# grayhong/self-diagnosing-gan

Measured on AMD Instinct MI355X. Metric: images/sec (G+D step), higher is better.
Workload: dtype f32

## Files before the change

### include/diagan_hip.h

```cpp
#ifndef DIAGAN_HIP_H
#define DIAGAN_HIP_H
#include <stddef.h>
#include <stdint.h>
#ifdef __cplusplus
extern "C" {
#endif

#define DIAGAN_OK 0
#define DIAGAN_EINVAL (-1)
#define DIAGAN_EHIP (-2)
#define DIAGAN_EUNSUP (-3)

const char* diagan_last_error(void);
int diagan_abi_version(void);
const char* diagan_target_arch(void);


int diagan_ldr_scores_f64(const double* rec, int T, int64_t N, int64_t row_stride, double* ldr,
                          double* ldrd, double* ldrv, double* ldrm, const double* t_vals, int n_t,
                          double* conf, double floor_val, double ratio, void* workspace,
                          void* stream);

int diagan_ldr_scores_f32(const float* rec, int T, int64_t N, int64_t row_stride, float* ldr,
                          float* ldrd, float* ldrv, float* ldrm, const float* t_vals, int n_t,
                          float* conf, float floor_val, float ratio, void* workspace, void* stream);

int diagan_logit_scatter(const float* logit, const int64_t* idx, int64_t n, void* rec_row,
                         int64_t N, int out_is_f64, int* oob_counter, void* stream);



int diagan_conv_gemm(const float* x, const float* w, float* y, const float* bias,
                     const float* residual, int res_relu, const float* mask_src, float mask_slope,
                     const float* pro_scale, const float* pro_shift, int pro_mode, float out_scale,
                     const float* scale0, const float* scale1, int scale_split,
                     int B, int Hi, int Wi, int Ci, int Ho, int Wo, int Co, int R, int S, int sy,
                     int dr, int off, int up, int Kp, int tile_cfg, float* splitk_ws, int64_t splitk_ws_floats,
                     float* stat_partials, int pro_group_rows, void* stream);
int diagan_conv_gemm_pick_ksplit(int M, int Co, int Kp, int cfg);

int diagan_conv3x3_co4_supported(int Ci, int Co, int R, int S, int sy, int dr, int off, int up);
int diagan_conv3x3_co4(const float* x, const float* w, float* y, const float* bias, const float* residual,
                       const float* pro_scale, const float* pro_shift, int pro_mode, int B, int H, int W, int Ci,
                       int dr, int off, int Kp, int group_imgs, void* stream);

int diagan_conv3x3_ci4_supported(int Ci, int Co, int R, int S, int sy, int dr, int off, int up);
int diagan_conv3x3_ci4(const float* x, const float* w, float* y, const float* bias, float out_scale, const float* scale0,
                       const float* scale1, int scale_split, int B, int H, int W, int Co, int Kp, void* stream);

int diagan_conv3x3_co4_wgrad_supported(int Ci, int Co, int R, int S, int sy, int dr, int off, int up);
int diagan_conv3x3_co4_wgrad_splits(int B, int H);
int diagan_conv3x3_co4_wgrad(const float* dy, const float* x, float* slab, int64_t slab_stride, int64_t bias_off,
                             const float* pro_scale, const float* pro_shift, int pro_mode, int B, int H, int W,
                             int Ci, int Kp, void* stream);

int diagan_conv_gemm_pick_cfg(int M, int Co, int Kp, int allow_split);
int diagan_conv_gemm_tile_rows(int cfg);
int diagan_conv_gemm_tile_cols(int cfg);
int diagan_conv_wino_supported(int Hi, int Wi, int Ci, int Ho, int Wo, int Co, int R, int S, int sy, int dr, int off,
                               int up);
int diagan_conv_wino_pool_supported(int B, int Hi, int Wi, int Ci, int Ho, int Wo, int Co, int R, int S, int sy, int dr,
                                    int off, int up, int pro_mode, int64_t ws_floats);
int diagan_conv_wino_unpool_supported(int B, int Hi, int Wi, int Ci, int Ho, int Wo, int Co, int R, int S, int sy, int dr,
                                      int off, int up, int64_t ws_floats);
int diagan_conv_gemm_set_wino(int mode);
int diagan_conv_gemm_get_wino(void);
int diagan_conv_gemm_set_wino4(int mode);
int diagan_conv_gemm_set_wino4x(int mode);
int diagan_conv_gemm_get_wino4x(void);
int diagan_conv_gemm_set_splitk_fused(int mode);
int diagan_conv_gemm_set_splitk_tickets(int* buf, int64_t slots);
typedef struct diagan_conv_opts {
  int32_t wino, wino4, wino4x, gemm_x3, gemm_x3b, splitk_fused, force_ksplit, tune;
  int32_t* tickets;
  int64_t ticket_slots;
} diagan_conv_opts;
int diagan_conv_gemm_next_opts(const diagan_conv_opts* opts);
int diagan_conv_gemm_pending_opts(diagan_conv_opts* opts);
int diagan_conv_gemm_last_cfg(void);
int diagan_conv_gemm_set_x3(int mode);
int diagan_conv_gemm_get_x3(void);
int diagan_conv_gemm_set_x3b(int mode);
int diagan_conv_gemm_get_x3b(void);
int diagan_conv_gemm_set_x3_pieces(int n);
int diagan_conv_gemm_get_x3_pieces(void);
int diagan_conv_gemm_x3b_force_form(int form);
int diagan_conv_gemm_out_map(int mul, int offy, int offx, int y0, int y1, int x0, int x1, int OH, int OW);
int diagan_conv_gemm_final_cfg(int B, int Hi, int Wi, int Ci, int Ho, int Wo, int Co, int R, int S, int sy, int dr, int off, int up,
                               int Kp, int allow_split, int64_t ws_floats, int pro_group_rows, int pro_mode, int plain_epilogue,
                               int want_stats);
int diagan_conv_wino4_pool_used(int B, int Ho, int Wo, int Ci, int Co, int64_t ws_floats);
int diagan_conv_wino4_upin_supported(int B, int Hi, int Wi, int Ci, int Ho, int Wo, int Co, int R, int S, int sy, int dr,
                                     int off, int up, int64_t ws_floats, int pro_group_rows);
int diagan_conv_gemm_weights_hint(const float* u, int kind, int flip, float scale);
int diagan_conv_gemm_last_weight_format(int* kind, int* flip, float* scale, int64_t* floats, int64_t* launches);
int64_t diagan_wino_weight_blocks(int Co, int Ci);
int diagan_wino_weights_batched(const void* jobs, int n, int blocks, void* stream);
int diagan_conv_gemm_pick_cfg_geom(int B, int Hi, int Wi, int Ci, int Ho, int Wo, int Co, int R, int S, int sy, int dr,
                                   int off, int up, int Kp, int allow_split, int64_t ws_floats);
int diagan_conv_gemm_pick_cfg_grouped(int B, int Hi, int Wi, int Ci, int Ho, int Wo, int Co, int R, int S, int sy, int dr,
                                      int off, int up, int Kp, int allow_split, int64_t ws_floats, int pro_group_rows);
int diagan_conv_gemm_set_stamp_buffer(unsigned long long* buf, int64_t slots);
int diagan_conv_gemm_tune(int force_ksplit, int flags, int lds_delta_bytes);

int diagan_conv_wgrad(const float* dy, const float* x, float* slab, int splits, int segments, int64_t slab_stride,
                      int64_t bias_off, const float* pro_scale, const float* pro_shift, int pro_mode, int B, int Hi, int Wi, int Ci, int Ho,
                      int Wo, int Co, int R, int S, int sy, int dr, int off, int up, int Kp,
                      void* stream);
int diagan_conv_wgrad_splits(int M, int Co, int Kp);
typedef struct {
  const float* dy;
  const float* x;
  float* slab;
  const float* pro_scale;
  const float* pro_shift;
  int64_t slab_stride, bias_off;
  int32_t splits, segments, pro_mode, B, Hi, Wi, Ci, Ho, Wo, Co, R, S, sy, dr, off, up, Kp, pad_;
} diagan_wgrad_job;
int diagan_conv_wgrad_batched(const diagan_wgrad_job* jobs, int n, void* stream);
int diagan_conv_wgrad_batch_max(void);
int diagan_conv_wgrad_batch_class(int Hi, int Wi, int Ci, int Ho, int Wo, int Co, int R, int S, int sy, int dr, int off, int up,
                                  int Kp, int pro_mode);
int diagan_conv_wgrad_uses_wino(int Hi, int Wi, int Ci, int Ho, int Wo, int Co, int R, int S, int sy, int dr, int off,
                                int up, int Kp);
int diagan_conv_wgrad_splits_geom(int B, int Hi, int Wi, int Ci, int Ho, int Wo, int Co, int R, int S, int sy, int dr,
                                  int off, int up, int Kp);
int diagan_conv_wgrad_uses_x3(int B, int Hi, int Wi, int Ci, int Ho, int Wo, int Co, int R, int S, int sy, int dr, int off,
                              int up, int Kp, int pro_mode, int64_t bias_off);
int diagan_conv_wgrad_set_x3(int on);

typedef struct {
  float* slab[2];
  const float* u[2];
  const float* v[2];
  const float* state[2];
  double* partials[2];
  float* grad;
  const float* W;
  int64_t stride;
  int splits, n_elem, n_w, Kp;
  int nctx, first_block;
} diagan_wgrad_layer;
int diagan_wgrad_finish_batched(const void* table_dev, int n_layers, int64_t total_blocks, int any_sn, void* stream);
int diagan_wgrad_finish_block_elems(int splits);

int diagan_wgrad_reduce(const float* slab, int splits, int64_t n_elem, float* out, int accumulate,
                        const float* w, double* dot_partials, void* stream);


int diagan_sn_power_iter(const float* W, float* u_buffer, float* sigma_buffer, float* u_out,
                         float* v_out, float* state, float* work, int Co, int Kp, float eps,
                         int update_buffers, void* stream);

typedef struct {
  const float* W;
  float* u_buf;
  float* sigma_buf;
  float* u_out;
  float* v_out;
  float* state;
  float* work;
  float* Wf;
  float* Wd;
  int Co, Ci, RS, Kp, Kd, pad;
} diagan_sn_layer;
int diagan_sn_prepare_batched(const void* table_dev, int n_layers, int max_Co, int max_Ci, int max_RS,
                              int max_Kp, float eps, int update_buffers, int write_wd, void* stream);
int diagan_pack_batched(const void* table_dev, int n_layers, int max_Co, int max_Ci, int max_RS, int write_wd,
                        void* stream);

int diagan_pack_weights(const float* W, const float* inv_sigma, float* Wf, float* Wd, int Co, int Ci,
                        int RS, int Kp, int Kd, void* stream);
int diagan_pack_oihw(const float* w, float scale, float* Wf, float* Wd, int Co_src, int Ci_src, int R, int S, int Co, int Ci, int Kp,
                     int Kd, void* stream);
int diagan_unpack_oihw(const float* gWp, float scale, float* gw, int Co_src, int Ci_src, int R, int S, int Ci, int Kp, void* stream);
int diagan_parity_weights(const float* w, float* buf, float* gw, int n, int R, int S, int C, int Kp, const int* kp, const int* off,
                          int adjoint, void* stream);


int diagan_sn_grad_fix(const float* G, const double* dot_partials, int nparts, const float* u,
                       const float* v, const float* state, float* grad, int Co, int Kp,
                       int accumulate, void* stream);


int diagan_nchw_to_nhwc(const float* src, float* dst, int B, int C, int H, int W, int Cp, void* stream);
int diagan_nhwc_to_nchw(const float* src, float* dst, int B, int C, int H, int W, int Cp, void* stream);

int diagan_tanh_fwd(const float* x, float* y, int64_t n, void* stream);
int diagan_tanh_bwd(const float* y, const float* g, float* gx, int64_t n, void* stream);

int64_t diagan_colred_workspace(int64_t M, int C);

int diagan_bn_stats(const float* x, int64_t M, int C, const float* gamma, const float* beta, float eps,
                    float momentum, float* running_mean, float* running_var, int training,
                    float* mean_out, float* invstd_out, float* scale_out, float* shift_out,
                    void* workspace, void* stream);
int diagan_bn_stats_grouped(const float* x, int64_t M, int C, int groups, const float* gamma, const float* beta, float eps,
                            float momentum, float* running_mean, float* running_var, float* mean_out, float* invstd_out,
                            float* scale_out, float* shift_out, void* workspace, void* stream);

int diagan_bn_stats_fused(const float* partials, int tiles, int64_t M, int C, const float* gamma, const float* beta,
                          float eps, float momentum, float* running_mean, float* running_var, float* mean_out,
                          float* invstd_out, float* scale_out, float* shift_out, int groups, double* workspace,
                          int64_t workspace_doubles, void* stream);
int diagan_bn_stats_fused_splits(int tiles, int C, int groups);

int diagan_bn_bwd(const float* g, const float* x, int64_t M, int C, const float* scale, const float* shift,
                  const float* mean, const float* invstd, int batch_stats, int relu, float slope,
                  const float* drop, float drop_scale, float* dgamma, float* dbeta,
                  int accumulate_param_grads, const float* residual, float* dx, float* coef,
                  void* workspace, void* stream);

int diagan_colsum(const float* x, int64_t M, int C, float* out, int accumulate, void* workspace, void* stream);

int diagan_upsample2x(const float* x, float* out, int B, int H, int W, int C, int pro_mode,
                      const float* scale, const float* shift, int group_imgs, void* stream);
int diagan_upsample2x_bwd(const float* g, float* out, int B, int H, int W, int C, const float* residual,
                          void* stream);

int diagan_avgpool2(const float* x, float* out, int B, int H, int W, int C, const float* residual, int relu_in,
                    void* stream);
int diagan_boxsum2(const float* x, float* out, int B, int H, int W, int C, int relu_in, void* stream);
int diagan_avgpool2_bwd(const float* g, float* out, int B, int H, int W, int C, const float* residual,
                        void* stream);

int diagan_head_fwd(const float* x, const float* w, const float* inv_sigma, const float* inv_sigma1, int split_b,
                    const float* bias, float* pooled, float* logit, int B, int HW, int C, void* stream);
int diagan_head_bwd(const float* dlogit, const float* w, const float* inv_sigma, const float* inv_sigma1, int split_b,
                    const float* x, const float* pooled, float* gx, float* G, double* dot, float* dbias,
                    int accumulate_bias, int B, int HW, int C, void* stream);

int diagan_act_fwd(const float* x, const float* scale, const float* shift, float slope, const float* drop, float drop_scale,
                   float* out, int64_t M, int C, void* stream);
int diagan_act_bwd(const float* g, const float* x, float slope, const float* drop, float drop_scale, float* out, int64_t n,
                   void* stream);
int diagan_linear1_fwd(const float* x, const float* w, const float* bias, float* logit, int B, int C, void* stream);
int diagan_linear1_wgrad(const float* dlogit, const float* x, float* dw, float* dbias, int B, int C, void* stream);
int diagan_linear1_bwd_input(const float* dlogit, const float* w, float* gx, int B, int C, void* stream);

int diagan_add(const float* a, const float* b, float* out, int64_t n, void* stream);


int diagan_loss_dis(const float* out_real, int n_real, const float* out_fake, int n_fake, int loss_type,
                    int gold, float* d_real, float* d_fake, float* out3, void* stream);
int diagan_loss_gen(const float* out_fake, int n, int k, int loss_type, float* d_fake, float* out1, void* stream);

int diagan_adam_step(float* p, const float* g, float* m, float* v, int64_t n, float lr, float beta1,
                     float beta2, float eps, float bias_correction1, float bias_correction2_sqrt, float grad_scale,
                     void* stream);
int diagan_adam_step_dev(float* p, const float* g, float* m, float* v, int64_t n, const float* hyper8, void* stream);

typedef struct diagan_ctx diagan_ctx;
int diagan_comm_unique_id(void* id128);
int diagan_ctx_create(diagan_ctx** out, const void* id128, int rank, int world, int device);
int diagan_ctx_destroy(diagan_ctx* ctx);
int diagan_ctx_rank(const diagan_ctx* ctx);
int diagan_ctx_world(const diagan_ctx* ctx);
int diagan_allreduce_grads(diagan_ctx* ctx, float* slab, int64_t n, void* stream);
int diagan_allgather_logits(diagan_ctx* ctx, const void* send, void* recv, int64_t n_per_rank, int elem_bytes,
                            void* stream);


int diagan_fused_bias_act(const float* x, const float* bias, const float* refer, float* out, int64_t n,
                          int64_t step_b, int size_b, int act, int grad, float alpha, float scale, void* stream);

int diagan_styled_bias_act(const float* x, const float* demod, const float* noise, const float* strength,
                           const float* bias, float* out, int B, int P, int C, int noise_per_image, float alpha,
                           float scale, void* stream);

int diagan_rowdot_chunks(int B, int P);
int diagan_rowdot(const float* a, const float* b, float* out, float* workspace, int B, int P, int C, void* stream);
int diagan_styled_bias_act_bwd(const float* gy, const float* y, const float* x, const float* demod, const float* noise,
                               float* gx, float* work_d, float* work_b, float* work_s, int B, int P, int C,
                               int noise_per_image, float alpha, float scale, void* stream);
int diagan_styled_bias_act_bwd_finish(const float* work_d, const float* work_b, const float* work_s, float* gd, float* gb, float* gs, int B,
                                      int P, int C, void* stream);

int diagan_small_linear_fwd(const float* x, const float* W, const float* bias, float* out, int B, int K, int C, float scale, float bias_mul,
                            void* stream);
int diagan_small_linear_bwd(const float* g, const float* x, const float* W, float* gW, float* gbias, float* gx, int B, int K, int C,
                            float scale, float bias_mul, void* stream);
int diagan_demod_fwd(const float* s, const float* w, float* d, float* wsq, int B, int Ci, int Co, int taps, float scale2, float eps,
                     void* stream);
int diagan_demod_bwd(const float* gd, const float* d, const float* s, const float* w, const float* wsq, float* gw, float* gs, int B, int Ci,
                     int Co, int taps, float scale2, void* stream);

int diagan_styled_bias_act_mod(const float* x, const float* demod, const float* noise, const float* strength, const float* bias,
                               const float* post, float* out, float* out_mod, int B, int P, int C, int noise_per_image, float alpha,
                               float scale, void* stream);
int diagan_styled_bias_act_mod_bwd(const float* gy, const float* gmod, const float* post, const float* y, const float* x,
                                   const float* demod, const float* noise, float* gx, float* work_d, float* work_b, float* work_s,
                                   float* work_p, int B, int P, int C, int noise_per_image, float alpha, float scale, void* stream);

int diagan_torgb_fwd(const float* x, const float* s, const float* w, const float* bias, float* out, int B, int P, int C, void* stream);
int diagan_torgb_bwd(const float* gy, const float* x, const float* s, const float* w, float* gx, float* work, float* gs, float* gw, int B,
                     int P, int C, void* stream);
int diagan_fromrgb_fwd(const float* x, const float* w, const float* bias, float* y, int B, int P, int C, float wscale, float alpha,
                       float scale, void* stream);
int diagan_fromrgb_bwd(const float* gy, const float* y, const float* x, const float* w, float* gx, float* work, int B, int P, int C,
                       float wscale, float alpha, float scale, void* stream);
int diagan_bias_act_fir(const float* input, const float* bias, const float* kernel, float* out, int major, int in_h, int in_w, int minor,
                        int kernel_h, int kernel_w, int pad_x0, int pad_x1, int pad_y0, int pad_y1, float alpha, float scale,
                        void* stream);
int diagan_bias_act_gate_bwd(const float* gy, const float* z, const float* bias, float* gx, float* work_b, int B, int P, int C,
                             float alpha, float scale, void* stream);
int diagan_fir_gate_bwd(const float* g, const float* kernel, const float* ref, const float* bias, float* gz, float* work_b, int major,
                        int in_h, int in_w, int minor, int kernel_h, int kernel_w, int pad_x0, int pad_x1, int pad_y0, int pad_y1,
                        float alpha, float scale, void* stream);
int diagan_upfirdn2d_add(const float* input, const float* kernel, const float* addend, float* out, int major, int in_h, int in_w, int minor,
                         int kernel_h, int kernel_w, int up_x, int up_y, int down_x, int down_y, int pad_x0, int pad_x1, int pad_y0,
                         int pad_y1, void* stream);
int diagan_bias_act_add(const float* x, const float* bias, const float* addend, float* out, int64_t n, int C, float alpha, float scale,
                        void* stream);
int diagan_fir_styled_act(const float* input, const float* kernel, float* out, int major, int in_h, int in_w, int minor, int kernel_h,
                          int kernel_w, int pad_x0, int pad_x1, int pad_y0, int pad_y1, const float* demod, const float* noise,
                          const float* strength, const float* bias, const float* post, int noise_per_image, float alpha, float scale,
                          void* stream);


int diagan_upfirdn2d(const float* input, const float* kernel, float* out, int major, int in_h, int in_w, int minor,
                     int kernel_h, int kernel_w, int up_x, int up_y, int down_x, int down_y, int pad_x0, int pad_x1,
                     int pad_y0, int pad_y1, int* out_h, int* out_w, void* stream);

int diagan_row_sqnorm(const float* x, float* out, int N, int D, int ld, void* stream);
int diagan_kth_smallest_rows(const float* T, const float* row_add, int rows, int cols, int ld, int k, float* out,
                             void* stream);
int diagan_any_lt_rows(const float* T, const float* row_add, const float* thr_col, const float* thr_row, int rows,
                       int cols, int ld, float* out, void* stream);
int diagan_any_lt_cols(const float* T, const float* row_add, const float* thr_col, const float* thr_row, int rows,
                       int cols, int ld, float* out, void* stream);

int diagan_gemm_f64(const double* A, const double* B, double* C, int M, int N, int K, int lda, int ldb, int ldc, int trans_a,
                    double alpha, double beta, double diag, double* trace_part, void* stream);
int diagan_gemm_f64_tile(void);
int diagan_sum_f64(const double* x, int64_t n, int square, double* out, void* stream);
int diagan_trace_f64(const double* S, int D, int ld, double* out, void* stream);
int diagan_sym_f64(double* S, int D, int ld, double scale, void* stream);
int diagan_scale_diag_f64(const double* src, double* dst, int D, int ld, double alpha, double d, void* stream);
int diagan_fid_term(const double* mu1, const double* mu2, const double* S1, const double* S2, int D, int ld, double* out,
                    void* stream);
int diagan_feat_colsum_chunks(int N);
int diagan_feat_moments(const void* x, int x_f64, int N, int D, int ld, double* mask, double* part, double* count, double* mean,
                        void* stream);
int diagan_feat_center(const void* x, int x_f64, const double* mask, const double* mean, int N, int D, int ld, double* xc, int ldc,
                       void* stream);
int diagan_moments_merge(double* n_run, double* mean_run, double* m2_run, int ld, const double* n_b, const double* mean_b,
                         const double* m2_b, int ldb, int D, void* stream);


int diagan_augment_params(void);
int diagan_augment_workspace(int B, int H, int W, int pad_x1, int pad_x2, int pad_y1, int pad_y2, int backward, int64_t* bytes);
int diagan_augment_forward(const float* img, const double* params, int B, int H, int W, int pad_x1, int pad_x2, int pad_y1,
                           int pad_y2, float* out, void* workspace, void* stream);
int diagan_augment_backward(const float* gout, const double* params, int B, int H, int W, int pad_x1, int pad_x2, int pad_y1,
                            int pad_y2, float* gimg, void* workspace, void* stream);

int diagan_incep_conv_kp(int R, int S, int Ci);
int diagan_incep_conv(const float* x, int B, int H, int W, int ctot_in, int c0_in, int Ci, const float* w, const float* bias, int Co,
                      int R, int S, int Kp, int stride_h, int stride_w, int pad_h, int pad_w, float* y, int Ho, int Wo, int ctot_out,
                      int c0_out, int relu, void* stream);
int diagan_incep_pool3(const float* x, int B, int H, int W, int ctot_in, int c0_in, int C, float* y, int Ho, int Wo, int ctot_out,
                       int c0_out, int mode, void* stream);
int diagan_incep_gap(const float* x, int B, int HW, int C, float* y, void* stream);
int diagan_incep_prep(const float* x, int nhwc, int B, int H, int W, float* y, int Ho, int Wo, int resize, float a, float b,
                      void* stream);

int diagan_poly_mmd_ws(int m);
int diagan_poly_mmd_sums(const void* X, int x_f64, int Nx, int ldx, const void* Y, int y_f64, int Ny, int ldy, const int* idx_x,
                         const int* idx_y, int S, int m, int D, int degree, double gamma, double coef0, double* ws, double* out,
                         void* stream);
int diagan_is_ws(int N, int C, int splits);
int diagan_is_scores(const float* logits, int N, int C, int ld, int splits, double* ws, double* out, void* stream);

int diagan_nn_argmin(const float* q, int Nq, int ldq, const float* c, int Nc, int ldc, const float* c_sqnorm, int D, long idx_offset,
                     int accumulate, float* best_t, long* best_idx, void* ws, void* stream);
size_t diagan_nn_argmin_ws(int Nq, int Nc);

#ifdef __cplusplus
}
#endif
#endif
```

### self-diagnosing-gan_amd/csrc/conv_gemm.hip

```cpp
#include "conv_common.h"
#include "switches.h"
#include <type_traits>
#include <stdlib.h>
#include <string.h>

extern "C" int diagan_conv_gemm_tile_rows(int cfg);
extern "C" int diagan_conv_gemm_tile_cols(int cfg);
extern "C" int diagan_conv_gemm_pick_ksplit(int M, int Co, int Kp, int cfg);
extern "C" int diagan_conv_gemm_pick_cfg_geom(int B, int Hi, int Wi, int Ci, int Ho, int Wo, int Co, int R, int S, int sy,
                                              int dr, int off, int up, int Kp, int allow_split, int64_t ws_floats);
extern "C" int diagan_conv_gemm_pick_cfg_grouped(int B, int Hi, int Wi, int Ci, int Ho, int Wo, int Co, int R, int S, int sy,
                                                 int dr, int off, int up, int Kp, int allow_split, int64_t ws_floats,
                                                 int pro_group_rows);
extern "C" int diagan_conv_wino_supported(int Hi, int Wi, int Ci, int Ho, int Wo, int Co, int R, int S, int sy, int dr,
                                          int off, int up);

namespace diagan {
int launch_gemm_x3(const ConvGemmArgs& a, float* ws, hipStream_t st);
bool gemm_x3_geom_ok(const ConvGemmArgs& a);
long gemm_x3_ws_floats(int Co, int Kp);
int launch_gemm_x3b(const ConvGemmArgs& a, const OutMap& map, float* ws, hipStream_t st);
bool gemm_x3b_geom_ok(const ConvGemmArgs& a);
long gemm_x3b_ws_floats(int Co, int Kp);
void gemm_x3b_force_form(int form);
int launch_wino(ConvGemmArgs a, float* ws, hipStream_t st);
long wino_ws_floats(int Co, int Ci);
int wino_ksplit(int B, int Ho, int Wo, int Ci, int Co, int allow_split, long ws_floats, int min_wgs);
int launch_wino4(ConvGemmArgs a, float* ws, hipStream_t st);
long wino4_ws_floats(int Co, int Ci);
bool wino4_geom_ok(int Ho, int Wo, int Ci);
int wino4_ksplit(int B, int Ho, int Wo, int Ci, int Co, int allow_split, long ws_floats);
bool wino4_pool_ok(int B, int Ho, int Wo, int Ci, int Co, long ws_floats, bool force);
int launch_wino4_pool(ConvGemmArgs a, float* ws, hipStream_t st);
int launch_wino4_unpool(ConvGemmArgs a, float* ws, hipStream_t st);
bool wino4_upin_ok(int B, int Ho, int Wo, int Ci, int Co, long ws_floats, bool force);
int launch_wino_weights_batched(const WinoJob* jobs, int n, int blocks, hipStream_t st);
int launch_wino4_upin(ConvGemmArgs a, float* ws, hipStream_t st);
void wino4_set_x3(int mode);
int wino4_get_x3();
int launch_wino_pool(ConvGemmArgs a, float* ws, hipStream_t st);
int launch_wino_unpool(ConvGemmArgs a, float* ws, hipStream_t st);
int wino_pool_ksplit(int B, int Ho, int Wo, int Ci, int Co, long slab_floats, int min_wgs);


template <int BM, int BN, int WM, int WN, int BK = 32, int PRO = -1, bool STAMP = false, bool FP = false, int KG = 1>
__global__ __launch_bounds__(256 * KG) void conv_gemm_kernel(const ConvGemmArgs a) {
  constexpr int CH = BK / 4;
  constexpr int RP = 256 / CH;
  constexpr int TM = BM / WM / 32, TN = BN / WN / 32;
  constexpr int AJ = BM / RP, BJ = BN / RP;
  auto swz = [](int row, int q) {
    return BK == 64 ? (q ^ (row & 15)) : BK == 32 ? (q ^ ((row >> 1) & 7)) : (q ^ ((row >> 2) & 3));
  };
  static_assert(WM * WN == 4, "4 waves");
  extern __shared__ __attribute__((aligned(16))) float smem_all[];
  constexpr int STAGE_FLOATS = 2 * (BM + BN) * BK;
  const int kg = KG > 1 ? __builtin_amdgcn_readfirstlane((int)threadIdx.x >> 8) : 0;
  float* const smem = smem_all + kg * STAGE_FLOATS;
  float* As = smem;
  float* Bs = smem + 2 * BM * BK;

  unsigned long long st_t[6] = {0, 0, 0, 0, 0, 0}, st_r0 = 0;
  auto stamp = [&](int i) {
    if constexpr (STAMP) {
      __builtin_amdgcn_sched_barrier(0);
      st_t[i] = __builtin_amdgcn_s_memtime();
      __builtin_amdgcn_sched_barrier(0);
    }
  };
  if constexpr (STAMP) st_r0 = __builtin_amdgcn_s_memrealtime();
  if (a.tune & 1) __builtin_amdgcn_s_setprio(3);
  stamp(0);
  const ConvGeom& g = a.g;
  const int pro_mode = PRO >= 0 ? PRO : a.pro_mode;
  const int tid = KG > 1 ? (threadIdx.x & 255) : threadIdx.x, lane = tid & 63, wave = tid >> 6;
  const int wm = wave / WN, wn = wave % WN;
  const int tiles_n = (g.Co + BN - 1) / BN;
  const int nwg = gridDim.x;
  const int tile = xcd_remap(blockIdx.x, nwg);
  const int m0 = (tile / tiles_n) * BM, n0 = (tile % tiles_n) * BN;

  const int lrow = tid / CH, lq = tid % CH;
  const int ush = g.up >> 1, upm = g.up - 1;
  const int pstep = (g.Ci * 4) >> ush;
  int base[AJ];
  unsigned vmask[AJ];
#pragma unroll
  for (int j = 0; j < AJ; ++j) {
    const int m = m0 + lrow + RP * j;
    base[j] = 0;
    vmask[j] = 0;
    if (m < a.M) {
      const unsigned t = fdiv((unsigned)m, a.dWo);
      const int ox = m - (int)t * g.Wo;
      const unsigned b = fdiv(t, a.dHo);
      const int oy = (int)t - (int)b * g.Ho;
      const int iy0 = oy * g.sy + g.off, ix0 = ox * g.sy + g.off;
      base[j] = (int)b * g.Hi * g.Wi * g.Ci * 4 + (iy0 * g.Wi + ix0) * pstep;
      unsigned mk = 0;
      if (g.up == 1) {
        const int ylo = g.dr > 0 ? max(0, -iy0) : max(0, iy0 - g.Hi + 1);
        const int yhi = g.dr > 0 ? min(g.R - 1, g.Hi - 1 - iy0) : min(g.R - 1, iy0);
        const int xlo = g.dr > 0 ? max(0, -ix0) : max(0, ix0 - g.Wi + 1);
        const int xhi = g.dr > 0 ? min(g.S - 1, g.Wi - 1 - ix0) : min(g.S - 1, ix0);
        if (yhi >= ylo) mk |= (2u << yhi) - (1u << ylo);
        if (xhi >= xlo) mk |= ((2u << xhi) - (1u << xlo)) << 16;
      } else {
        for (int r = 0; r < g.R; ++r) {
          const int yn = iy0 + r * g.dr;
          if (yn >= 0 && (yn & upm) == 0 && (yn >> ush) < g.Hi) mk |= 1u << r;
        }
        for (int q = 0; q < g.S; ++q) {
          const int xn = ix0 + q * g.dr;
          if (xn >= 0 && (xn & upm) == 0 && (xn >> ush) < g.Wi) mk |= 0x10000u << q;
        }
      }
      vmask[j] = mk;
    }
  }
  const int nk_all = g.Kp / BK;
  const int k_per = (nk_all + a.ksplit * KG - 1) / (a.ksplit * KG);
  const int k_begin = min((int)(blockIdx.y * KG + kg) * k_per, nk_all), k_end = min(k_begin + k_per, nk_all);
  int kc, kr, ks;
  {
    const int kflat = k_begin * BK + lq * 4, tap = kflat / g.Ci;
    kc = kflat - tap * g.Ci;
    kr = tap / g.S;
    ks = tap - kr * g.S;
  }
  const int rowstep = g.dr * g.Wi * pstep, colstep = g.dr * pstep;

  const __amdgpu_buffer_rsrc_t xsrc = __builtin_amdgcn_make_buffer_rsrc(
      const_cast<float*>(a.x), 0, (int)((unsigned)g.B * g.Hi * g.Wi * g.Ci * 4u), 0x00020000);
  const __amdgpu_buffer_rsrc_t wsrc = __builtin_amdgcn_make_buffer_rsrc(
      const_cast<float*>(a.w), 0, (int)((unsigned)g.Co * g.Kp * 4u), 0x00020000);
  const bool affine = pro_mode == PRO_AFFINE_RELU || pro_mode == PRO_AFFINE;
  const int pro_group_off = a.pro_group_rows > 0 ? (m0 / a.pro_group_rows) * g.Ci : 0;
  unsigned wbase[BJ];
#pragma unroll
  for (int j = 0; j < BJ; ++j) wbase[j] = ((unsigned)(n0 + lrow + RP * j) * g.Kp + lq * 4) * 4u;

  f32x4 ra[AJ], rb[BJ], psc = {1.f, 1.f, 1.f, 1.f}, psh = {0.f, 0.f, 0.f, 0.f};
  unsigned a_ok = 0;

  const bool ut = (g.Ci % BK) == 0;
  int ukr = 0, uks = 0, ukc = 0;
  unsigned avo[AJ], tap_ok = 0;
  auto tap_setup = [&]() {
    const int toff = ukr * rowstep + uks * colstep + lq * 16;
    const int r_ = min(ukr, 15), s_ = 16 + uks;
    tap_ok = 0;
#pragma unroll
    for (int j = 0; j < AJ; ++j) {
      const unsigned okb = (vmask[j] >> r_) & (vmask[j] >> s_) & 1u;
      avo[j] = (unsigned)(base[j] + toff) | ((okb ^ 1u) << 31);
      tap_ok |= okb << j;
    }
  };
  if (ut) {
    const int kflat0 = k_begin * BK, tap0 = kflat0 / g.Ci;
    ukc = kflat0 - tap0 * g.Ci;
    ukr = tap0 / g.S;
    uks = tap0 - ukr * g.S;
    tap_setup();
  }
  const float* const pro_sc_lane = a.pro_scale ? a.pro_scale + pro_group_off + lq * 4 : nullptr;
  const float* const pro_sh_lane = a.pro_shift ? a.pro_shift + pro_group_off + lq * 4 : nullptr;

  int tapoff = 0, krs = 0, kss = 0;
  auto load_piece = [&](int kk, int p, auto utc) {
    if constexpr (decltype(utc)::value) {
      if (p == 0) {
        a_ok = tap_ok;
        if (affine) {
          psc = *reinterpret_cast<const f32x4*>(pro_sc_lane + ukc);
          psh = *reinterpret_cast<const f32x4*>(pro_sh_lane + ukc);
        }
      }
      if (p < AJ) {
        ra[p] = __builtin_bit_cast(f32x4, __builtin_amdgcn_raw_buffer_load_b128(xsrc, avo[p], ukc * 4, 0));
      } else {
        rb[p - AJ] = __builtin_bit_cast(f32x4, __builtin_amdgcn_raw_buffer_load_b128(wsrc, wbase[p - AJ], kk * (BK * 4), 0));
      }
      if (p == AJ + BJ - 1) {
        ukc += BK;
        if (ukc >= g.Ci) {
          ukc = 0;
          if (++uks == g.S) {
            uks = 0;
            ++ukr;
          }
          tap_setup();
        }
      }
      return;
    }
    if (p == 0) {
      tapoff = kr * rowstep + ks * colstep + kc * 4;
      krs = min(kr, 15);
      kss = 16 + ks;
      a_ok = 0;
      if (affine) {
        const int kcs = min(kc, g.Ci - 4);
        psc = *reinterpret_cast<const f32x4*>(a.pro_scale + pro_group_off + kcs);
        psh = *reinterpret_cast<const f32x4*>(a.pro_shift + pro_group_off + kcs);
      }
    }
    if (p < AJ) {
      const int j = p;
      const unsigned okb = (vmask[j] >> krs) & (vmask[j] >> kss) & 1u;
      const unsigned off = (unsigned)(base[j] + tapoff) | ((okb ^ 1u) << 31);
      ra[j] = __builtin_bit_cast(f32x4, __builtin_amdgcn_raw_buffer_load_b128(xsrc, off, 0, 0));
      a_ok |= okb << j;
    } else {
      const int j = p - AJ;
      rb[j] = __builtin_bit_cast(f32x4, __builtin_amdgcn_raw_buffer_load_b128(wsrc, wbase[j] + (unsigned)kk * (BK * 4u), 0, 0));
    }
    if (p == AJ + BJ - 1) {
      kc += BK;
      if (g.Ci >= BK) {
        const bool w = kc >= g.Ci;
        kc -= w ? g.Ci : 0;
        ks += w ? 1 : 0;
        const bool r = ks == g.S;
        ks = r ? 0 : ks;
        kr += r ? 1 : 0;
      } else {
        const int kflat = (kk + 1) * BK + lq * 4, tap = kflat / g.Ci;
        kc = kflat - tap * g.Ci;
        kr = tap / g.S;
        ks = tap - kr * g.S;
      }
    }
  };
  auto load_tiles = [&](int kk) {
    if (ut) {
#pragma unroll
      for (int p = 0; p < AJ + BJ; ++p) load_piece(kk, p, std::true_type{});
    } else {
#pragma unroll
      for (int p = 0; p < AJ + BJ; ++p) load_piece(kk, p, std::false_type{});
    }
  };
  auto store_piece = [&](int buf, int p) {
    if (p < AJ) {
      const int j = p;
      const int row = lrow + RP * j;
      f32x4 v = ra[j];
      if (pro_mode != PRO_NONE) {
        if (affine) v = v * psc + psh;
        if (pro_mode == PRO_LRELU) {
#pragma unroll
          for (int e = 0; e < 4; ++e) v[e] = v[e] > 0.f ? v[e] : 0.2f * v[e];
        } else if (pro_mode != PRO_AFFINE) {
#pragma unroll
          for (int e = 0; e < 4; ++e) v[e] = fmaxf(v[e], 0.f);
        }
        if (affine) {
          const float keep = (float)((a_ok >> j) & 1u);
          v *= keep;
        }
      }
      *reinterpret_cast<f32x4*>(As + buf * BM * BK + row * BK + (swz(row, lq) << 2)) = v;
    } else {
      const int j = p - AJ;
      const int row = lrow + RP * j;
      *reinterpret_cast<f32x4*>(Bs + buf * BN * BK + row * BK + (swz(row, lq) << 2)) = rb[j];
    }
  };
  auto store_tiles = [&](int buf) {
#pragma unroll
    for (int p = 0; p < AJ + BJ; ++p) store_piece(buf, p);
  };

  f32x16 acc[TM][TN];
#pragma unroll
  for (int i = 0; i < TM; ++i)
#pragma unroll
    for (int j = 0; j < TN; ++j)
#pragma unroll
      for (int e = 0; e < 16; ++e) acc[i][j][e] = 0.f;

  const int fi = lane & 31, fh = lane >> 5;
  int fao[BK / 8], fbo[BK / 8];
#pragma unroll
  for (int u = 0; u < BK / 8; ++u) {
    const int ra_ = wm * (TM * 32) + fi, rb_ = wn * (TN * 32) + fi;
    fao[u] = ra_ * BK + (swz(ra_, 2 * u + fh) << 2);
    fbo[u] = 2 * BM * BK + rb_ * BK + (swz(rb_, 2 * u + fh) << 2);
  }
  const int sto = lrow * BK + (swz(lrow, lq) << 2);

  stamp(1);
  if (k_begin < k_end) {
    load_tiles(k_begin);
    store_tiles(0);
  }
  __syncthreads();

  constexpr int NE = (BK / 8) * 4, NP = AJ + BJ;
  constexpr int PPE = (2 * NP + NE - 1) / NE;
  constexpr int LE = (NP + PPE - 1) / PPE;
  static_assert(2 * LE <= NE, "load and store pieces of a tile must not share an e-step");
  auto kstep = [&](int kk, auto has_next) {
    const int cur = (kk - k_begin) & 1;
    const float* Ac = As + cur * BM * BK;
    const float* Bc = Bs + cur * BN * BK;
    f32x4 fa[2][TM], fb[2][TN];
    auto read_frags = [&](int slot, int u) {
      const int q = 2 * u + fh;
#pragma unroll
      for (int i = 0; i < TM; ++i) {
        const int row = wm * (TM * 32) + i * 32 + fi;
        fa[slot][i] = *reinterpret_cast<const f32x4*>(Ac + row * BK + (swz(row, q) << 2));
      }
#pragma unroll
      for (int j = 0; j < TN; ++j) {
        const int row = wn * (TN * 32) + j * 32 + fi;
        fb[slot][j] = *reinterpret_cast<const f32x4*>(Bc + row * BK + (swz(row, q) << 2));
      }
    };
    if constexpr (FP) read_frags(0, 0);
#pragma unroll
    for (int u = 0; u < BK / 8; ++u) {
      const int fs = FP ? (u & 1) : 0;
      if constexpr (FP) {
        if (u + 1 < BK / 8) read_frags((u + 1) & 1, u + 1);
      } else {
        read_frags(0, u);
      }
#pragma unroll
      for (int e = 0; e < 4; ++e) {
        const int es = u * 4 + e;
        if (decltype(has_next)::value && es < LE) {
#pragma unroll
          for (int pp = 0; pp < PPE; ++pp)
            if (es * PPE + pp < NP) load_piece(kk + 1, es * PPE + pp, std::false_type{});
        }
        if (decltype(has_next)::value && es >= NE - LE) {
          __builtin_amdgcn_sched_barrier(0);
#pragma unroll
          for (int pp = 0; pp < PPE; ++pp)
            if ((es - (NE - LE)) * PPE + pp < NP) store_piece(cur ^ 1, (es - (NE - LE)) * PPE + pp);
        }
#pragma unroll
        for (int i = 0; i < TM; ++i)
#pragma unroll
          for (int j = 0; j < TN; ++j)
            acc[i][j] = __builtin_amdgcn_mfma_f32_32x32x2f32(fa[fs][i][e], fb[fs][j][e], acc[i][j], 0, 0, 0);
      }
    }
    __syncthreads();
  };
  auto kstep_u = [&](int kk, auto curc, auto has_next) {
    constexpr int cur = decltype(curc)::value;
    f32x4 fa[2][TM], fb[2][TN];
    auto read_frags = [&](int slot, int u) {
#pragma unroll
      for (int i = 0; i < TM; ++i) fa[slot][i] = *reinterpret_cast<const f32x4*>(smem + fao[u] + cur * BM * BK + i * 32 * BK);
#pragma unroll
      for (int j = 0; j < TN; ++j) fb[slot][j] = *reinterpret_cast<const f32x4*>(smem + fbo[u] + cur * BN * BK + j * 32 * BK);
    };
    auto store_piece_u = [&](int p) {
      if (p < AJ) {
        f32x4 v = ra[p];
        if (pro_mode != PRO_NONE) {
          if (affine) v = v * psc + psh;
          if (pro_mode == PRO_LRELU) {
#pragma unroll
            for (int e = 0; e < 4; ++e) v[e] = v[e] > 0.f ? v[e] : 0.2f * v[e];
          } else if (pro_mode != PRO_AFFINE) {
#pragma unroll
            for (int e = 0; e < 4; ++e) v[e] = fmaxf(v[e], 0.f);
          }
          if (affine) {
            const float keep = (float)((a_ok >> p) & 1u);
            v *= keep;
          }
        }
        *reinterpret_cast<f32x4*>(smem + sto + (cur ^ 1) * BM * BK + p * RP * BK) = v;
      } else {
        *reinterpret_cast<f32x4*>(smem + sto + 2 * BM * BK + (cur ^ 1) * BN * BK + (p - AJ) * RP * BK) = rb[p - AJ];
      }
    };
    if constexpr (FP) read_frags(0, 0);
#pragma unroll
    for (int u = 0; u < BK / 8; ++u) {
      const int fs = FP ? (u & 1) : 0;
      if constexpr (FP) {
        if (u + 1 < BK / 8) read_frags((u + 1) & 1, u + 1);
      } else {
        read_frags(0, u);
      }
#pragma unroll
      for (int e = 0; e < 4; ++e) {
        const int es = u * 4 + e;
        if (decltype(has_next)::value && es < LE) {
#pragma unroll
          for (int pp = 0; pp < PPE; ++pp)
            if (es * PPE + pp < NP) load_piece(kk + 1, es * PPE + pp, std::true_type{});
        }
        if (decltype(has_next)::value && es >= NE - LE) {
          __builtin_amdgcn_sched_barrier(0);
#pragma unroll
          for (int pp = 0; pp < PPE; ++pp)
            if ((es - (NE - LE)) * PPE + pp < NP) store_piece_u((es - (NE - LE)) * PPE + pp);
        }
#pragma unroll
        for (int i = 0; i < TM; ++i)
#pragma unroll
          for (int j = 0; j < TN; ++j)
            acc[i][j] = __builtin_amdgcn_mfma_f32_32x32x2f32(fa[fs][i][e], fb[fs][j][e], acc[i][j], 0, 0, 0);
      }
    }
    __syncthreads();
  };
  if (a.tune & 1) __builtin_amdgcn_s_setprio(0);
  stamp(2);
  if (ut) {
    const std::integral_constant<int, 0> b0;
    const std::integral_constant<int, 1> b1;
    int kk = k_begin;
    for (; kk + 2 < k_end; kk += 2) {
      kstep_u(kk, b0, std::true_type{});
      kstep_u(kk + 1, b1, std::true_type{});
    }
    if (kk + 1 < k_end) {
      kstep_u(kk, b0, std::true_type{});
      kstep_u(kk + 1, b1, std::false_type{});
    } else if (kk < k_end) {
      kstep_u(kk, b0, std::false_type{});
    }
  } else {
    for (int kk = k_begin; kk + 1 < k_end; ++kk) kstep(kk, std::true_type{});
    if (k_begin < k_end) kstep(k_end - 1, std::false_type{});
  }
  stamp(3);
  if (a.tune & 2) __builtin_amdgcn_s_setprio(3);
  if constexpr (KG > 1) {
    if (kg > 0) {
#pragma unroll
      for (int i = 0; i < TM; ++i)
#pragma unroll
        for (int j = 0; j < TN; ++j)
#pragma unroll
          for (int e = 0; e < 16; ++e) smem[((i * TN + j) * 16 + e) * 256 + tid] = acc[i][j][e];
    }
    __syncthreads();
    if (kg > 0) return;
#pragma unroll
    for (int q = 1; q < KG; ++q)
#pragma unroll
      for (int i = 0; i < TM; ++i)
#pragma unroll
        for (int j = 0; j < TN; ++j)
#pragma unroll
          for (int e = 0; e < 16; ++e) acc[i][j][e] += smem_all[q * STAGE_FLOATS + ((i * TN + j) * 16 + e) * 256 + tid];
    static_assert(TM * TN * 16 * 256 <= STAGE_FLOATS, "the accumulators of a K-group fit its stage region");
  }

  const float sc0 = a.scale0 ? a.scale0[0] : a.out_scale, sc1 = a.scale1 ? a.scale1[0] : a.out_scale;
  const int split = a.scale0 ? a.scale_split : 0x7fffffff;
  const unsigned rowbytes = (unsigned)g.Co * 4u;
  const unsigned ybytes = (unsigned)a.M * rowbytes;
  float* ydst = a.ksplit > 1 ? a.slab + (long)blockIdx.y * a.M * g.Co : a.y;
  const __amdgpu_buffer_rsrc_t ysrc = __builtin_amdgcn_make_buffer_rsrc(ydst, 0, (int)ybytes, 0x00020000);
  const __amdgpu_buffer_rsrc_t rsrc = __builtin_amdgcn_make_buffer_rsrc(
      const_cast<float*>(a.residual ? a.residual : a.y), 0, a.residual ? (int)ybytes : 0, 0x00020000);
  const __amdgpu_buffer_rsrc_t msrc = __builtin_amdgcn_make_buffer_rsrc(
      const_cast<float*>(a.mask_src ? a.mask_src : a.y), 0, a.mask_src ? (int)ybytes : 0, 0x00020000);
  const float rfloor = a.res_relu ? 0.f : -__builtin_huge_valf();
  float cs1[TN], cs2[TN];
#pragma unroll
  for (int j = 0; j < TN; ++j) cs1[j] = cs2[j] = 0.f;
  auto epilogue = [&](auto has_res, auto has_mask, auto has_stats, auto raw) {
#pragma unroll
    for (int i = 0; i < TM; ++i) {
#pragma unroll
      for (int j = 0; j < TN; ++j) {
        const int n = n0 + wn * (TN * 32) + j * 32 + fi;
        const bool col_ok = n < g.Co;
        const float bv = (!decltype(raw)::value && a.bias && col_ok) ? a.bias[n] : 0.f;
        const int mrow = m0 + wm * (TM * 32) + i * 32 + 4 * fh;
        const unsigned vbase = col_ok ? ((unsigned)mrow * g.Co + n) * 4u : 0x80000000u;
        float rres[16], rmsk[16];
        if (decltype(has_res)::value) {
#pragma unroll
          for (int e = 0; e < 16; ++e)
            rres[e] = __builtin_bit_cast(float, __builtin_amdgcn_raw_buffer_load_b32(
                                                    rsrc, vbase, (int)(((e & 3) + 8 * (e >> 2)) * rowbytes), 0));
        }
        if (decltype(has_mask)::value) {
#pragma unroll
          for (int e = 0; e < 16; ++e)
            rmsk[e] = __builtin_bit_cast(float, __builtin_amdgcn_raw_buffer_load_b32(
                                                    msrc, vbase, (int)(((e & 3) + 8 * (e >> 2)) * rowbytes), 0));
        }
#pragma unroll
        for (int e = 0; e < 16; ++e) {
          const int k = (e & 3) + 8 * (e >> 2);
          const int soff = (int)(k * rowbytes);
          const float av = acc[i][j][e];
          if (decltype(raw)::value) {
            __builtin_amdgcn_raw_buffer_store_b32(__float_as_uint(av), ysrc, vbase, soff, 0);
            continue;
          }
          const int m = mrow + k;
          float v = fmaf(av, m < split ? sc0 : sc1, bv);
          if (decltype(has_res)::value) v += fmaxf(rres[e], rfloor);
          if (decltype(has_mask)::value) v = rmsk[e] > 0.f ? v : v * a.mask_slope;
          __builtin_amdgcn_raw_buffer_store_b32(__float_as_uint(v), ysrc, vbase, soff, 0);
          if (decltype(has_stats)::value) {
            const float vm = (m < a.M && col_ok) ? v : 0.f;
            cs1[j] += vm;
            cs2[j] = fmaf(vm, vm, cs2[j]);
          }
        }
      }
    }
  };
  {
    using T = std::true_type;
    using F = std::false_type;
    const bool hr = a.residual != nullptr, hm = a.mask_src != nullptr, hs = a.stat_partials != nullptr;
    if (a.ksplit > 1) epilogue(F{}, F{}, F{}, T{});
    else if (hs) { if (hr) epilogue(T{}, F{}, T{}, F{}); else epilogue(F{}, F{}, T{}, F{}); }
    else if (hr && hm) epilogue(T{}, T{}, F{}, F{});
    else if (hr) epilogue(T{}, F{}, F{}, F{});
    else if (hm) epilogue(F{}, T{}, F{}, F{});
    else epilogue(F{}, F{}, F{}, F{});
  }
  if (a.stat_partials) {
    float* red = smem;
#pragma unroll
    for (int j = 0; j < TN; ++j) {
      cs1[j] += __shfl_xor(cs1[j], 32, 64);
      cs2[j] += __shfl_xor(cs2[j], 32, 64);
      if (fh == 0) {
        const int col = wn * (TN * 32) + j * 32 + fi;
        red[(wm * BN + col) * 2 + 0] = cs1[j];
        red[(wm * BN + col) * 2 + 1] = cs2[j];
      }
    }
    __syncthreads();
    if (tid < BN && n0 + tid < g.Co) {
      float t1 = 0.f, t2 = 0.f;
#pragma unroll
      for (int w = 0; w < WM; ++w) { t1 += red[(w * BN + tid) * 2]; t2 += red[(w * BN + tid) * 2 + 1]; }
      float* p = a.stat_partials + (long)(tile / tiles_n) * 2 * g.Co;
      p[n0 + tid] = t1;
      p[g.Co + n0 + tid] = t2;
    }
  }
  if constexpr (STAMP) {
    stamp(4);
    asm volatile("s_waitcnt vmcnt(0)" ::: "memory");
    stamp(5);
    if (tid == 0 && a.stamps) {
      unsigned long long* o = a.stamps + ((size_t)blockIdx.y * gridDim.x + blockIdx.x) * 8;
      o[0] = st_r0;
      o[1] = __builtin_amdgcn_s_memrealtime();
      for (int i = 0; i < 5; ++i) o[2 + i] = st_t[i + 1] - st_t[i];
      o[7] = (unsigned long long)__builtin_amdgcn_s_getreg((31 << 11) | 4) |
             ((unsigned long long)__builtin_amdgcn_s_getreg((31 << 11) | 20) << 32);
    }
  }
}

__global__ __launch_bounds__(256) void splitk_epilogue_kernel(const ConvGemmArgs a) {
  const int C4 = a.g.Co >> 2;
  const long n4 = (long)a.M * C4;
  const float sc0 = a.scale0 ? a.scale0[0] : 1.f, sc1 = a.scale1 ? a.scale1[0] : 1.f;
  for (long i = (long)blockIdx.x * 256 + threadIdx.x; i < n4; i += (long)gridDim.x * 256) {
    const int c4 = (int)(i % C4);
    const int m = (int)(i / C4);
    f32x4 s = reinterpret_cast<const f32x4*>(a.slab)[i];
    for (int k = 1; k < a.ksplit; ++k) s += reinterpret_cast<const f32x4*>(a.slab)[(long)k * n4 + i];
    const float sc = a.scale0 ? (m < a.scale_split ? sc0 : sc1) : a.out_scale;
    s *= sc;
    if (a.bias) s += reinterpret_cast<const f32x4*>(a.bias)[c4];
    if (a.residual) {
      f32x4 r;
      if (a.res_up == 1) {
        const int ox = m % a.g.Wo, q = m / a.g.Wo, oy = q % a.g.Ho, b = q / a.g.Ho;
        r = residual_up2(a.residual, b, oy, ox, a.g.Ho >> 1, a.g.Wo >> 1, a.g.Co, c4 * 4);
      } else if (a.res_up == 2) {
        const int ox = m % a.g.Wo, q = m / a.g.Wo, oy = q % a.g.Ho, b = q / a.g.Ho;
        r = 0.25f * *reinterpret_cast<const f32x4*>(a.residual + (((long)b * (a.g.Ho >> 1) + (oy >> 1)) * (a.g.Wo >> 1) + (ox >> 1)) * a.g.Co + c4 * 4);
      } else {
        r = reinterpret_cast<const f32x4*>(a.residual)[i];
      }
      if (a.res_relu) {
#pragma unroll
        for (int e = 0; e < 4; ++e) r[e] = fmaxf(r[e], 0.f);
      }
      s += r;
    }
    if (a.mask_src) {
      const f32x4 ms = reinterpret_cast<const f32x4*>(a.mask_src)[i];
#pragma unroll
      for (int e = 0; e < 4; ++e) s[e] = ms[e] > 0.f ? s[e] : s[e] * a.mask_slope;
    }
    reinterpret_cast<f32x4*>(a.y)[i] = s;
  }
}

static unsigned long long* g_stamps = nullptr;
static long g_stamp_slots = 0;
static int g_force_ksplit = 0;
static int g_tune_flags = -1;
static long g_lds_delta = 0;
static int g_wino = -1;
static int g_wino4 = -1;
struct WinoFormat { const float* u; int kind, flip; float scale; long floats; };
static thread_local WinoFormat g_hint_next = {nullptr, 0, 0, 0.f, 0}, g_hint_now = {nullptr, 0, 0, 0.f, 0}, g_fmt_last = {nullptr, 0, 0, 0.f, 0};
static thread_local long g_weight_launches = 0;
constexpr int kDefaultTune = 0;

static int g_gemm_x3 = -1;
static int g_gemm_x3b = -1;
static int x3b_min_tiles() { return kGemmX3bMinTiles.env(); }
static thread_local OutMap g_map_next = {0, 0, 0, 0, 0, 0, 0, 0, 0};
struct CallOpts {
  int wino, wino4, wino4x, gemm_x3, gemm_x3b, splitk_fused, force_ksplit, tune;
  int* tickets;
  long ticket_slots;
};
static const CallOpts kNoOpts = {-1, -1, -1, -1, -1, -1, 0, -1, nullptr, 0};
static thread_local CallOpts g_opts_next = kNoOpts, g_opts_now = kNoOpts;
static thread_local int g_last_cfg = 0;
int call_opt_wino4x() { return g_opts_now.wino4x; }
static int sel_wino() { return kWino.get(g_opts_now.wino, g_wino); }
static int sel_wino4() { return g_opts_now.wino4 >= 0 ? g_opts_now.wino4 : g_wino4; }
static int sel_force_ksplit() { return g_opts_now.force_ksplit > 0 ? g_opts_now.force_ksplit : g_force_ksplit; }
static bool gemm_x3_on() { return kGemmX3.get(g_opts_now.gemm_x3, g_gemm_x3) != 0; }
static bool gemm_x3b_on() { return kGemmX3b.get(g_opts_now.gemm_x3b, g_gemm_x3b) != 0; }
static bool x3b_takes(const ConvGemmArgs& a, int cfg, int64_t ws_floats) {
  if (!gemm_x3b_on() || !(cfg == 1 || cfg == 3 || cfg == 5 || cfg == 7 || cfg == 8)) return false;
  const ConvGeom& g = a.g;
  return gemm_x3b_geom_ok(a) && g.Kp >= 128 && g.Co >= 64 && (long)cdiv(a.M, 128) * cdiv(g.Co, 128) >= x3b_min_tiles() &&
         (double)a.M * g.Co * g.Kp >= 4e9 && gemm_x3b_ws_floats(g.Co, g.Kp) <= ws_floats;
}
static int g_splitk_fused = -1;
static int* g_tickets = nullptr;
static long g_ticket_slots = 0;
static int* splitk_tickets(long tiles) {
  if (!kSplitkFused.get(g_opts_now.splitk_fused, g_splitk_fused)) return nullptr;
  if (g_opts_now.tickets) return tiles <= g_opts_now.ticket_slots ? g_opts_now.tickets : nullptr;
  return (g_tickets && tiles <= g_ticket_slots) ? g_tickets : nullptr;
}

static int splitk_second_stage(const ConvGemmArgs& a, hipStream_t st, const char* what) {
  long blocks = ((long)a.M * (a.g.Co / 4) + 255) / 256;
  if (blocks > 4096) blocks = 4096;
  hipLaunchKernelGGL(splitk_epilogue_kernel, dim3((int)blocks), dim3(256), 0, st, a);
  return check_launch(what);
}

template <int BM, int BN, int WM, int WN, int BK, int PRO, bool STAMP = false, bool FP = false, int KG = 1>
static int launch_one(const ConvGemmArgs& a, hipStream_t st) {
  const int tiles = cdiv(a.M, BM) * cdiv(a.g.Co, BN);
  const size_t lds = (size_t)((long)((size_t)2 * KG * (BM + BN) * BK * sizeof(float)) + g_lds_delta);
  auto kern = conv_gemm_kernel<BM, BN, WM, WN, BK, PRO, STAMP, FP, KG>;
  static FuncAttrLatch latch;
  DG_LDS(latch, kern, lds);
  hipLaunchKernelGGL(kern, dim3(tiles, a.ksplit), dim3(256 * KG), lds, st, a);
  return a.ksplit > 1 ? splitk_second_stage(a, st, "conv_gemm") : check_launch("conv_gemm");
}

template <int BM, int BN, int WM, int WN, int BK = 32, bool SPEC = false, bool FP = false, int KG = 1>
static int launch_cfg(const ConvGemmArgs& a, hipStream_t st) {
  if (a.stamps && KG > 1) return set_err(DIAGAN_EUNSUP, "conv_gemm: no stamped build of the two-group kernel");
  if (a.stamps) {
    if (a.pro_mode == PRO_NONE) return launch_one<BM, BN, WM, WN, BK, PRO_NONE, true, FP>(a, st);
    if (a.pro_mode == PRO_RELU) return launch_one<BM, BN, WM, WN, BK, PRO_RELU, true, FP>(a, st);
    return set_err(DIAGAN_EUNSUP, "conv_gemm: the stamped diagnostic kernels exist for prologue modes 0 and 1");
  }
  if (SPEC)
    return with_pro(a.pro_mode, [&](auto pro) { return launch_one<BM, BN, WM, WN, BK, SPEC ? decltype(pro)::value : -1, false, FP, KG>(a, st); });
  return launch_one<BM, BN, WM, WN, BK, -1, false, FP, KG>(a, st);
}

}

using namespace diagan;

static bool split128_enabled() { return kSplit128.env() > 0; }

DIAGAN_API int diagan_conv_gemm_pick_cfg(int M, int Co, int Kp, int allow_split) {
  const int small = 7;
  if (Kp <= 256) return small;
  const long t128 = (long)cdiv(M, 128) * cdiv(Co, 128), t64 = (long)cdiv(M, 64) * cdiv(Co, 64);
  if (split128_enabled() && allow_split && (Co & 127) == 0 && t128 <= 256 && diagan_conv_gemm_pick_ksplit(M, Co, Kp, 1) > 1) return 1;
  if (Co <= 64 && Kp >= 256) return M >= 65536 ? 5 : (M >= 32768 ? 8 : 7);
  const long s128 = 256 * 2, s64 = 256 * 4;
  const double q128 = (double)t128 / (double)(cdiv(t128, s128) * s128);
  const double q64 = (double)t64 / (double)(cdiv(t64, s64) * s64);
  const double waste128 = (double)M * Co / ((double)t128 * 128 * 128);
  const double waste64 = (double)M * Co / ((double)t64 * 64 * 64);
  const double bias = 1.08;
  if (bias * q128 * waste128 > q64 * waste64) return 1;
  if (kKg2.env() && t64 <= 256 && Kp >= 16 * 32 && diagan_conv_gemm_pick_ksplit(M, Co, Kp, small) == 1) return 14;
  return small;
}

DIAGAN_API int diagan_conv_gemm_pick_ksplit(int M, int Co, int Kp, int cfg) {
  const int forced = sel_force_ksplit() > 0 ? sel_force_ksplit() : kKsplit.env();
  if (forced > 0 && !(Co & 3)) return forced < Kp / 64 ? forced : (Kp / 64 > 0 ? Kp / 64 : 1);
  if (Co & 3) return 1;
  const int nk = Kp / 32;
  if (cfg == 1) {
    if (!split128_enabled()) return 1;
    const long t128 = (long)cdiv(M, 128) * cdiv(Co, 128);
    if (t128 > 256 || nk < 64) return 1;
    int s = t128 <= 128 ? 4 : 2;
    while (s > 1 && nk / s < 16) --s;
    return s;
  }
  if (cfg != 3 && cfg != 7) return 1;
  const long tiles = (long)cdiv(M, 64) * cdiv(Co, 64);
  if (nk < 16) return 1;
  if (tiles <= 320) {
    if (nk < 64) return 1;
    int s = nk / 24;
    return s > 4 ? 4 : s;
  }
  if (tiles > 512) return 1;
  long sp = 1024 / tiles;
  if (sp > nk / 8) sp = nk / 8;
  return sp < 2 ? 1 : (int)sp;
}

const float* diagan::wino_weights_ready(int kind, int flip, float scale, long floats) {
  g_fmt_last = WinoFormat{nullptr, kind, flip, scale, floats};
  if (g_hint_now.u && g_hint_now.kind == kind && g_hint_now.flip == flip && g_hint_now.scale == scale) return g_hint_now.u;
  ++g_weight_launches;
  return nullptr;
}

DIAGAN_API int diagan_conv_gemm_weights_hint(const float* u, int kind, int flip, float scale) {
  g_hint_next = WinoFormat{u, kind, flip, scale, 0};
  return DIAGAN_OK;
}
DIAGAN_API int diagan_conv_gemm_last_weight_format(int* kind, int* flip, float* scale, int64_t* floats, int64_t* launches) {
  if (kind) *kind = g_fmt_last.kind;
  if (flip) *flip = g_fmt_last.flip;
  if (scale) *scale = g_fmt_last.scale;
  if (floats) *floats = g_fmt_last.floats;
  if (launches) *launches = g_weight_launches;
  return DIAGAN_OK;
}
DIAGAN_API int64_t diagan_wino_weight_blocks(int Co, int Ci) { return (int64_t)cdiv(Ci, 32) * cdiv(Co, 64); }
DIAGAN_API int diagan_wino_weights_batched(const void* jobs, int n, int blocks, void* stream) {
  DG_REQUIRE(jobs && n > 0 && blocks > 0, "wino_weights_batched: bad job table");
  return launch_wino_weights_batched((const WinoJob*)jobs, n, blocks, (hipStream_t)stream);
}

DIAGAN_API int diagan_conv_gemm(const float* x, const float* w, float* y, const float* bias,
                                const float* residual, int res_relu, const float* mask_src, float mask_slope,
                                const float* pro_scale, const float* pro_shift, int pro_mode,
                                float out_scale, const float* scale0, const float* scale1, int scale_split,
                                int B, int Hi, int Wi, int Ci, int Ho, int Wo, int Co,
                                int R, int S, int sy, int dr, int off, int up, int Kp, int tile_cfg,
                                float* splitk_ws, int64_t splitk_ws_floats, float* stat_partials, int pro_group_rows,
                                void* stream) {
  g_hint_now = g_hint_next;
  g_hint_next = WinoFormat{nullptr, 0, 0, 0.f, 0};
  g_fmt_last = WinoFormat{nullptr, 0, 0, 0.f, 0};
  const OutMap map = g_map_next;
  g_map_next = OutMap{0, 0, 0, 0, 0, 0, 0, 0, 0};
  struct OptsScope {
    OptsScope() { g_opts_now = g_opts_next; g_opts_next = kNoOpts; }
    ~OptsScope() { g_opts_now = kNoOpts; }
  } opts_scope;
  g_last_cfg = 0;
  DG_REQUIRE(x && w && y, "conv_gemm: null tensor");
  DG_REQUIRE(B > 0 && Hi > 0 && Wi > 0 && Ho > 0 && Wo > 0 && Co > 0 && R > 0 && S > 0, "conv_gemm: bad dims");
  DG_REQUIRE(Ci > 0 && (Ci & 3) == 0, "conv_gemm: Ci=%d must be a positive multiple of 4 (pad the tensor)", Ci);
  DG_REQUIRE(up == 1 || up == 2, "conv_gemm: up=%d unsupported (1 or 2)", up);
  DG_REQUIRE(dr == 1 || dr == -1, "conv_gemm: dr must be +-1");
  DG_REQUIRE(R <= 15 && S <= 15, "conv_gemm: filter %dx%d larger than 15x15", R, S);
  DG_REQUIRE(Kp % 32 == 0 && Kp >= R * S * Ci, "conv_gemm: Kp=%d must be a multiple of 32 and >= R*S*Ci=%d", Kp, R * S * Ci);
  DG_REQUIRE(pro_mode >= 0 && pro_mode <= 4, "conv_gemm: bad pro_mode %d", pro_mode);
  DG_REQUIRE(!(pro_mode == PRO_AFFINE_RELU || pro_mode == PRO_AFFINE) || (pro_scale && pro_shift),
             "conv_gemm: affine prologue needs scale/shift");
  DG_REQUIRE((long)B * Ho * Wo * Co * 4 < (1L << 31) && (long)B * Hi * Wi * Ci * 4 < (1L << 31) &&
                 (long)Co * Kp * 4 < (1L << 31),
             "conv_gemm: tensors must be smaller than 2 GiB (32-bit buffer offsets)");
  ConvGemmArgs a;
  a.x = x; a.w = w; a.y = y; a.bias = bias; a.residual = residual; a.mask_src = mask_src;
  a.pro_scale = pro_scale; a.pro_shift = pro_shift; a.mask_slope = mask_slope; a.out_scale = out_scale;
  a.scale0 = scale0; a.scale1 = scale1; a.scale_split = scale_split;
  DG_REQUIRE(!scale0 || scale1, "conv_gemm: scale0 and scale1 must be given together");
  DG_REQUIRE(!(stat_partials && mask_src), "conv_gemm: stat_partials (forward statistics) and mask_src (backward mask) are exclusive");
  a.pro_mode = pro_mode; a.M = B * Ho * Wo; a.res_relu = res_relu & 1; a.res_up = (res_relu & 2) ? 1 : (res_relu & 4) ? 2 : 0;
  DG_REQUIRE((res_relu & ~7) == 0 && (res_relu & 6) != 6, "conv_gemm: res_relu=%d (bit 0: relu(residual), bit 1: half-resolution residual, "
             "up-sampled; bit 2: half-resolution residual, un-pooled)", res_relu);
  DG_REQUIRE(a.res_up != 1 || (residual && !(Ho & 1) && !(Wo & 1) && !mask_src && !a.res_relu),
             "conv_gemm: a half-resolution residual needs the tensor, even Ho / Wo, no backward mask and no ReLU on it");
  DG_REQUIRE(a.res_up != 2 || (residual && !(Ho & 1) && !(Wo & 1) && !a.res_relu && !stat_partials),
             "conv_gemm: an un-pooled half-resolution residual needs the tensor, even Ho / Wo, no ReLU on it, no statistics");
  a.g = ConvGeom{B, Hi, Wi, Ci, Ho, Wo, Co, R, S, sy, dr, off, up, R * S * Ci, Kp};
  a.dWo = make_fastdiv((unsigned)Wo);
  a.dHo = make_fastdiv((unsigned)Ho);
  a.stat_partials = stat_partials;
  a.pro_group_rows = pro_group_rows;
  hipStream_t st = (hipStream_t)stream;
  int cfg = tile_cfg != 0 ? tile_cfg
                          : diagan_conv_gemm_pick_cfg_grouped(B, Hi, Wi, Ci, Ho, Wo, Co, R, S, sy, dr, off, up, Kp,
                                                              (splitk_ws && !stat_partials) ? 1 : 0,
                                                              splitk_ws ? splitk_ws_floats : 0, pro_group_rows);
  if (tile_cfg == 0 && splitk_ws && x3b_takes(a, cfg, splitk_ws_floats)) cfg = 17;
  g_last_cfg = cfg;
  if (map.mul != 0) {
    DG_REQUIRE(map.mul > 0 && map.OH > 0 && map.OW > 0 && map.y0 >= 0 && map.x0 >= 0 && map.y1 <= Ho && map.x1 <= Wo &&
                   map.offy >= 0 && map.offx >= 0 && (map.y1 <= map.y0 || map.mul * (map.y1 - 1 - map.y0) + map.offy < map.OH) &&
                   (map.x1 <= map.x0 || map.mul * (map.x1 - 1 - map.x0) + map.offx < map.OW) &&
                   (long)B * map.OH * map.OW * Co * 4 < (1L << 31),
               "conv_gemm: output map (mul %d, off %d/%d, window [%d,%d) x [%d,%d), target %d x %d) does not fit", map.mul, map.offy,
               map.offx, map.y0, map.y1, map.x0, map.x1, map.OH, map.OW);
    DG_REQUIRE(cfg == 17, "conv_gemm: an output map is written by the split-operand kernel only (tile_cfg 17; ask "
               "diagan_conv_gemm_final_cfg first)");
  }
  const int bm = diagan_conv_gemm_tile_rows(cfg);
  DG_REQUIRE(bm > 0, "conv_gemm: unknown tile_cfg %d (0 = auto, 1 = 128x128, 3 = 64x64, 5 = 256x64, 7 = 64x64 with fragment "
             "prefetch, 8 = 128x64 with fragment prefetch, 9 = Winograd F(2x2,3x3), 11 / 12 = Winograd + average pool and its data-gradient, 13 = Winograd F(4x4,3x3), 15 = the same on the bilinear x2 of a half-resolution input; 2, 4, 6, 10 were retired)", tile_cfg);
  DG_REQUIRE(pro_group_rows >= 0 && (pro_group_rows == 0 || (pro_group_rows % bm == 0 && a.M % pro_group_rows == 0)),
             "conv_gemm: pro_group_rows=%d must be a multiple of the %d-row tile and divide M=%d", pro_group_rows, bm, a.M);
  a.slab = splitk_ws;
  a.tickets = nullptr;
  a.ksplit = 1;
  a.tune = first_set(g_opts_now.tune, g_tune_flags, kDefaultTune);
  a.stamps = nullptr;
  if (g_stamps) {
    const long wgs = (long)cdiv(a.M, bm) * cdiv(Co, diagan_conv_gemm_tile_cols(cfg)) * 16;
    DG_REQUIRE(wgs <= g_stamp_slots, "conv_gemm: stamp buffer has %ld slots, this launch may need %ld", g_stamp_slots, wgs);
    a.stamps = g_stamps;
  }
  if (splitk_ws && !stat_partials) {
    const int ks = diagan_conv_gemm_pick_ksplit(a.M, Co, Kp, cfg);
    if (ks > 1 && (int64_t)ks * a.M * Co <= splitk_ws_floats) a.ksplit = ks;
  }
  if (cfg == 11) {
    DG_REQUIRE(diagan_conv_wino_supported(Hi, Wi, Ci, Ho, Wo, Co, R, S, sy, dr, off, up) && dr == 1 && Co % 64 == 0 &&
                   (pro_mode == PRO_NONE || pro_mode == PRO_RELU) && !mask_src && !stat_partials && !a.res_up && pro_group_rows == 0,
               "conv_gemm: tile_cfg 11 (Winograd + average pool) needs a forward 3x3 / stride 1 / pad 1 geometry with even H, W, "
               "Ci %% 8 == 0, Co %% 64 == 0, prologue none / ReLU, no mask, statistics or half-resolution residual");
    if (sel_wino4() != 0 && splitk_ws && wino4_pool_ok(B, Ho, Wo, Ci, Co, (long)splitk_ws_floats, sel_wino4() == 2)) {
      a.ksplit = 1;
      return launch_wino4_pool(a, splitk_ws, st);
    }
    const long wfl = wino_ws_floats(Co, Ci);
    DG_REQUIRE(splitk_ws && splitk_ws_floats >= wfl, "conv_gemm: tile_cfg 11 needs %ld floats of workspace for the transformed weights", wfl);
    int ks = wino_pool_ksplit(B, Ho, Wo, Ci, Co, (long)splitk_ws_floats - wfl, 192);
    if (ks < 1) ks = 1;
    a.ksplit = ks;
    a.slab = splitk_ws + wfl;
    int rc = launch_wino_pool(a, splitk_ws, st);
    if (rc == DIAGAN_OK && ks > 1) {
      ConvGemmArgs e = a;
      e.M = B * (Ho >> 1) * (Wo >> 1);
      e.scale_split = a.scale_split >> 2;
      e.out_scale = a.out_scale;
      rc = splitk_second_stage(e, st, "conv_wino_pool split-K epilogue");
    }
    return rc;
  }
  if (cfg == 12) {
    DG_REQUIRE(diagan_conv_wino_supported(Hi, Wi, Ci, Ho, Wo, Co, R, S, sy, dr, off, up) && dr == -1 && Co % 64 == 0 &&
                   pro_mode == PRO_NONE && !stat_partials && !a.res_up && pro_group_rows == 0,
               "conv_gemm: tile_cfg 12 (data-gradient through an average pool, Winograd) needs the data-gradient geometry of a "
               "3x3 / stride 1 / pad 1 layer with even H, W, Ci %% 8 == 0, Co %% 64 == 0, no prologue, statistics or half-resolution residual");
    if (sel_wino4() != 0 && splitk_ws && wino4_pool_ok(B, Ho, Wo, Ci, Co, (long)splitk_ws_floats, sel_wino4() == 2)) {
      a.ksplit = 1;
      return launch_wino4_unpool(a, splitk_ws, st);
    }
    const long wfl = wino_ws_floats(Co, Ci);
    DG_REQUIRE(splitk_ws && splitk_ws_floats >= wfl, "conv_gemm: tile_cfg 12 needs %ld floats of workspace for the transformed weights", wfl);
    long slab_tiles = ((long)splitk_ws_floats - wfl) / 4;
    int ks = wino_pool_ksplit(B, Ho, Wo, Ci, Co, slab_tiles, 192);
    if (ks < 1) ks = 1;
    a.ksplit = ks;
    a.slab = splitk_ws + wfl;
    int rc = launch_wino_unpool(a, splitk_ws, st);
    if (rc == DIAGAN_OK && ks > 1) rc = splitk_second_stage(a, st, "conv_wino_unpool split-K epilogue");
    return rc;
  }
  if (cfg == 15) {
    DG_REQUIRE(diagan_conv_wino_supported(Hi, Wi, Ci, Ho, Wo, Co, R, S, sy, dr, off, up) && dr == 1 && wino4_geom_ok(Ho, Wo, Ci) &&
                   !mask_src && (pro_group_rows == 0 || pro_group_rows % 512 == 0),
               "conv_gemm: tile_cfg 15 (Winograd F(4x4,3x3) on an up-sampled input) needs a forward 3x3 / stride 1 / pad 1 geometry, "
               "H and W multiples of 4, Ci %% 8 == 0, no backward mask, prologue groups of whole 512-row tiles");
    const long wfl = wino4_ws_floats(Co, Ci);
    DG_REQUIRE(splitk_ws && splitk_ws_floats >= wfl, "conv_gemm: tile_cfg 15 needs %ld floats of workspace for the transformed weights", wfl);
    a.ksplit = 1;
    return launch_wino4_upin(a, splitk_ws, st);
  }
  if (cfg == 13) {
    DG_REQUIRE(diagan_conv_wino_supported(Hi, Wi, Ci, Ho, Wo, Co, R, S, sy, dr, off, up) && wino4_geom_ok(Ho, Wo, Ci),
               "conv_gemm: tile_cfg 13 (Winograd F(4x4,3x3)) needs a 3x3 / stride 1 / pad 1 geometry, H and W multiples of 4, Ci %% 8 == 0");
    const long wfl = wino4_ws_floats(Co, Ci);
    DG_REQUIRE(splitk_ws && splitk_ws_floats >= wfl, "conv_gemm: tile_cfg 13 needs %ld floats of workspace for the transformed weights", wfl);
    int ks = 1;
    if (tile_cfg == 0 && !stat_partials) {
      ks = wino4_ksplit(B, Ho, Wo, Ci, Co, 1, (long)splitk_ws_floats);
      if (ks < 1) ks = 1;
    } else if (sel_force_ksplit() > 1 && !stat_partials && wfl + (long)sel_force_ksplit() * a.M * Co <= splitk_ws_floats && Ci / 8 / sel_force_ksplit() >= 1) {
      ks = sel_force_ksplit();
    }
    a.ksplit = ks;
    a.slab = splitk_ws + wfl;
    int rc = launch_wino4(a, splitk_ws, st);
    if (rc == DIAGAN_OK && ks > 1) rc = splitk_second_stage(a, st, "conv_wino4 split-K epilogue");
    return rc;
  }
  if (cfg == 9) {
    DG_REQUIRE(diagan_conv_wino_supported(Hi, Wi, Ci, Ho, Wo, Co, R, S, sy, dr, off, up),
               "conv_gemm: tile_cfg 9 (Winograd F(2x2,3x3)) needs a 3x3 / stride 1 / pad 1 geometry, even H and W, Ci %% 8 == 0");
    DG_REQUIRE(splitk_ws && splitk_ws_floats >= wino_ws_floats(Co, Ci),
               "conv_gemm: tile_cfg 9 needs %ld floats of workspace for the transformed weights", wino_ws_floats(Co, Ci));
    const long wfl = wino_ws_floats(Co, Ci);
    int ks = 1;
    if (tile_cfg == 0 && !stat_partials) {
      ks = wino_ksplit(B, Ho, Wo, Ci, Co, 1, (long)splitk_ws_floats, 192);
      if (ks < 1) ks = 1;
    } else if (sel_force_ksplit() > 1 && !stat_partials && wfl + (long)sel_force_ksplit() * a.M * Co <= splitk_ws_floats &&
               Ci / 16 / sel_force_ksplit() >= 1) {
      ks = sel_force_ksplit();
    }
    a.ksplit = ks;
    a.slab = splitk_ws + wfl;
    if (ks > 1) a.tickets = splitk_tickets((long)cdiv(a.M / 4, 64) * cdiv(Co, 64));
    int rc = launch_wino(a, splitk_ws, st);
    if (rc == DIAGAN_OK && ks > 1 && !a.tickets) rc = splitk_second_stage(a, st, "conv_wino split-K epilogue");
    return rc;
  }
  DG_REQUIRE(!a.res_up, "conv_gemm: a half-resolution residual is added by the Winograd kernel only (tile_cfg 9; ask "
             "diagan_conv_gemm_pick_cfg_geom first)");
  if (cfg == 16 || (cfg == 14 && tile_cfg == 0 && R == 3 && S == 3 && gemm_x3_on() && gemm_x3_geom_ok(a) && splitk_ws &&
                    gemm_x3_ws_floats(Co, Kp) <= splitk_ws_floats)) {
    DG_REQUIRE(gemm_x3_geom_ok(a) && splitk_ws && gemm_x3_ws_floats(Co, Kp) <= splitk_ws_floats,
               "conv_gemm: tile_cfg 16 (split-operand implicit GEMM) needs stride 1, no up-sampling, Ci %% 32 == 0, an even number of "
               "32-channel K-steps, Kp == R*S*Ci, prologue none / ReLU, no statistics, and %ld floats of workspace", gemm_x3_ws_floats(Co, Kp));
    a.ksplit = 1;
    g_last_cfg = 16;
    return launch_gemm_x3(a, splitk_ws, st);
  }
  if (cfg == 17) {
    DG_REQUIRE(gemm_x3b_geom_ok(a) && splitk_ws && gemm_x3b_ws_floats(Co, Kp) <= splitk_ws_floats,
               "conv_gemm: tile_cfg 17 (split-operand implicit GEMM, 128 x 128 tiles) needs a gather without up-sampling, Ci %% 32 == 0, "
               "Kp == R*S*Ci, prologue none / ReLU / leaky ReLU, a plain epilogue (out_scale, bias, residual) and %ld floats of workspace",
               gemm_x3b_ws_floats(Co, Kp));
    a.ksplit = 1;
    return launch_gemm_x3b(a, map, splitk_ws, st);
  }
  switch (cfg) {
    case 1: return launch_cfg<128, 128, 2, 2, 32, true>(a, st);
    case 3: return launch_cfg<64, 64, 2, 2, 32, true>(a, st);
    case 5: return launch_cfg<256, 64, 4, 1, 32, true>(a, st);
    case 7: return launch_cfg<64, 64, 2, 2, 32, true, true>(a, st);
    case 8: return launch_cfg<128, 64, 2, 2, 32, true, true>(a, st);
    case 14: return launch_cfg<64, 64, 2, 2, 32, true, true, 2>(a, st);
    default: return set_err(DIAGAN_EINVAL, "conv_gemm: unknown tile_cfg %d", tile_cfg);
  }
}

DIAGAN_API int diagan_conv_gemm_tile_rows(int cfg) {
  switch (cfg) { case 1: case 8: case 17: return 128; case 3: case 7: case 14: case 16: return 64; case 5: case 9: case 11: case 12: return 256; case 13: case 15: return 512; default: return 0; }
}
DIAGAN_API int diagan_conv_gemm_tile_cols(int cfg) {
  switch (cfg) { case 1: case 11: case 12: case 17: return 128; case 3: case 5: case 7: case 8: case 9: case 13: case 14: case 15: case 16: return 64; default: return 0; }
}

DIAGAN_API int diagan_conv_wino_supported(int Hi, int Wi, int Ci, int Ho, int Wo, int Co, int R, int S, int sy, int dr,
                                          int off, int up) {
  return R == 3 && S == 3 && sy == 1 && up == 1 && ((dr == 1 && off == -1) || (dr == -1 && off == 1)) && Hi == Ho &&
         Wi == Wo && !(Ho & 1) && !(Wo & 1) && (Ci & 7) == 0 && (Co & 3) == 0;
}

DIAGAN_API int diagan_conv_wino_pool_supported(int B, int Hi, int Wi, int Ci, int Ho, int Wo, int Co, int R, int S, int sy,
                                               int dr, int off, int up, int pro_mode, int64_t ws_floats) {
  const int wino = sel_wino();
  if (!wino || !kWinoPool.env() || dr != 1 || Co % 64 != 0 || Ci < 16 || !(pro_mode == PRO_NONE || pro_mode == PRO_RELU)) return 0;
  if (!diagan_conv_wino_supported(Hi, Wi, Ci, Ho, Wo, Co, R, S, sy, dr, off, up)) return 0;
  const long wfl = wino_ws_floats(Co, Ci);
  if (ws_floats < wfl) return 0;
  return wino_pool_ksplit(B, Ho, Wo, Ci, Co, (long)ws_floats - wfl, 192) > 0 ? 1 : 0;
}

DIAGAN_API int diagan_conv_wino_unpool_supported(int B, int Hi, int Wi, int Ci, int Ho, int Wo, int Co, int R, int S, int sy,
                                                 int dr, int off, int up, int64_t ws_floats) {
  const int wino = sel_wino();
  if (!wino || !kWinoPool.env() || dr != -1 || Co % 64 != 0 || Ci < 16) return 0;
  if (!diagan_conv_wino_supported(Hi, Wi, Ci, Ho, Wo, Co, R, S, sy, dr, off, up)) return 0;
  const long wfl = wino_ws_floats(Co, Ci);
  if (ws_floats < wfl) return 0;
  return wino_pool_ksplit(B, Ho, Wo, Ci, Co, ((long)ws_floats - wfl) / 4, 192) > 0 ? 1 : 0;
}

static int pick_cfg_geom_impl(int B, int Hi, int Wi, int Ci, int Ho, int Wo, int Co, int R, int S, int sy, int dr, int off,
                              int up, int Kp, int allow_split, int64_t ws_floats, bool allow_w4);
DIAGAN_API int diagan_conv_gemm_pick_cfg_geom(int B, int Hi, int Wi, int Ci, int Ho, int Wo, int Co, int R, int S, int sy,
                                              int dr, int off, int up, int Kp, int allow_split, int64_t ws_floats) {
  return pick_cfg_geom_impl(B, Hi, Wi, Ci, Ho, Wo, Co, R, S, sy, dr, off, up, Kp, allow_split, ws_floats, true);
}
static int pick_cfg_geom_impl(int B, int Hi, int Wi, int Ci, int Ho, int Wo, int Co, int R, int S, int sy, int dr, int off,
                              int up, int Kp, int allow_split, int64_t ws_floats, bool allow_w4) {
  const int wino = sel_wino();
  if (wino && diagan_conv_wino_supported(Hi, Wi, Ci, Ho, Wo, Co, R, S, sy, dr, off, up) &&
      ws_floats >= wino_ws_floats(Co, Ci) && Ci >= 16) {
    const int wsplit = kWinoSplit.env();
    if (allow_w4 && kWino4.env() && sel_wino4() != 0 && wino4_geom_ok(Ho, Wo, Ci) && Ci >= kWino4MinCi.env() && ws_floats >= wino4_ws_floats(Co, Ci) &&
        wino4_ksplit(B, Ho, Wo, Ci, Co, wsplit ? allow_split : 0, (long)ws_floats) > 0)
      return 13;
    if (wino_ksplit(B, Ho, Wo, Ci, Co, wsplit ? allow_split : 0, (long)ws_floats, kWinoMinWgs.env()) > 0) return 9;
  }
  return diagan_conv_gemm_pick_cfg(B * Ho * Wo, Co, Kp, allow_split);
}

DIAGAN_API int diagan_conv_gemm_pick_cfg_grouped(int B, int Hi, int Wi, int Ci, int Ho, int Wo, int Co, int R, int S, int sy,
                                                 int dr, int off, int up, int Kp, int allow_split, int64_t ws_floats,
                                                 int pro_group_rows) {
  int cfg = diagan_conv_gemm_pick_cfg_geom(B, Hi, Wi, Ci, Ho, Wo, Co, R, S, sy, dr, off, up, Kp, allow_split, ws_floats);
  if (cfg == 13 && pro_group_rows > 0 && pro_group_rows % 512 != 0)
    cfg = pick_cfg_geom_impl(B, Hi, Wi, Ci, Ho, Wo, Co, R, S, sy, dr, off, up, Kp, allow_split, ws_floats, false);
  if (pro_group_rows > 0 && pro_group_rows % diagan_conv_gemm_tile_rows(cfg) != 0) {
    cfg = diagan_conv_gemm_pick_cfg(B * Ho * Wo, Co, Kp, allow_split);
    if (pro_group_rows % diagan_conv_gemm_tile_rows(cfg) != 0) cfg = 3;
  }
  return cfg;
}

DIAGAN_API int diagan_conv_gemm_get_wino(void) { return g_wino; }
DIAGAN_API int diagan_conv_gemm_set_wino(int mode) {
  DG_REQUIRE(mode >= -1 && mode <= 1, "set_wino: -1, 0 or 1");
  g_wino = mode;
  return DIAGAN_OK;
}

DIAGAN_API int diagan_conv_wino4_pool_used(int B, int Ho, int Wo, int Ci, int Co, int64_t ws_floats) {
  return sel_wino4() != 0 && wino4_pool_ok(B, Ho, Wo, Ci, Co, (long)ws_floats, sel_wino4() == 2) ? 1 : 0;
}

DIAGAN_API int diagan_conv_wino4_upin_supported(int B, int Hi, int Wi, int Ci, int Ho, int Wo, int Co, int R, int S, int sy, int dr,
                                                int off, int up, int64_t ws_floats, int pro_group_rows) {
  const int wino = sel_wino();
  if (!wino || sel_wino4() == 0 || dr != 1 || !diagan_conv_wino_supported(Hi, Wi, Ci, Ho, Wo, Co, R, S, sy, dr, off, up)) return 0;
  if (pro_group_rows > 0 && pro_group_rows % 512 != 0) return 0;
  return wino4_upin_ok(B, Ho, Wo, Ci, Co, (long)ws_floats, sel_wino4() == 2) ? 1 : 0;
}

DIAGAN_API int diagan_conv_gemm_set_wino4(int mode) {
  DG_REQUIRE(mode >= -1 && mode <= 2, "set_wino4: -1, 0, 1 or 2 (2: also the pooled launches of any size -- tests)");
  g_wino4 = mode;
  return DIAGAN_OK;
}

DIAGAN_API int diagan_conv_gemm_set_wino4x(int mode) {
  DG_REQUIRE(mode >= -1 && mode <= 1, "set_wino4x: -1, 0 or 1");
  wino4_set_x3(mode);
  return DIAGAN_OK;
}
DIAGAN_API int diagan_conv_gemm_get_wino4x(void) { return wino4_get_x3(); }
DIAGAN_API int diagan_conv_gemm_set_x3(int mode) {
  DG_REQUIRE(mode >= -1 && mode <= 1, "set_x3: -1, 0 or 1");
  g_gemm_x3 = mode;
  return DIAGAN_OK;
}
DIAGAN_API int diagan_conv_gemm_get_x3(void) { return gemm_x3_on() ? 1 : 0; }
DIAGAN_API int diagan_conv_gemm_set_x3b(int mode) {
  DG_REQUIRE(mode >= -1 && mode <= 1, "set_x3b: -1, 0 or 1");
  g_gemm_x3b = mode;
  return DIAGAN_OK;
}
DIAGAN_API int diagan_conv_gemm_get_x3b(void) { return gemm_x3b_on() ? 1 : 0; }
namespace diagan { void x3_set_pieces(int n); int x3_pieces(); }
DIAGAN_API int diagan_conv_gemm_set_x3_pieces(int n) {
  diagan::x3_set_pieces(n);
  return DIAGAN_OK;
}
DIAGAN_API int diagan_conv_gemm_get_x3_pieces(void) { return diagan::x3_pieces(); }
DIAGAN_API int diagan_conv_gemm_x3b_force_form(int form) {
  DG_REQUIRE(form >= 0 && form <= 2, "x3b_force_form: 0, 1 or 2");
  gemm_x3b_force_form(form);
  return DIAGAN_OK;
}
DIAGAN_API int diagan_conv_gemm_out_map(int mul, int offy, int offx, int y0, int y1, int x0, int x1, int OH, int OW) {
  g_map_next = OutMap{mul, offy, offx, y0, y1, x0, x1, OH, OW};
  return DIAGAN_OK;
}
DIAGAN_API int diagan_conv_gemm_final_cfg(int B, int Hi, int Wi, int Ci, int Ho, int Wo, int Co, int R, int S, int sy, int dr,
                                          int off, int up, int Kp, int allow_split, int64_t ws_floats, int pro_group_rows,
                                          int pro_mode, int plain_epilogue, int want_stats) {
  struct PendingScope {
    CallOpts saved;
    PendingScope() : saved(g_opts_now) { g_opts_now = g_opts_next; }
    ~PendingScope() { g_opts_now = saved; }
  } pending_scope;
  int cfg = diagan_conv_gemm_pick_cfg_grouped(B, Hi, Wi, Ci, Ho, Wo, Co, R, S, sy, dr, off, up, Kp, allow_split, ws_floats,
                                              pro_group_rows);
  ConvGemmArgs a = {};
  a.pro_mode = pro_mode;
  a.M = B * Ho * Wo;
  a.g = ConvGeom{B, Hi, Wi, Ci, Ho, Wo, Co, R, S, sy, dr, off, up, R * S * Ci, Kp};
  a.pro_group_rows = pro_group_rows;
  static float dummy;
  a.stat_partials = want_stats ? &dummy : nullptr;
  a.mask_src = plain_epilogue ? nullptr : &dummy;
  if (ws_floats > 0 && x3b_takes(a, cfg, ws_floats)) return 17;
  a.mask_src = nullptr;
  if (cfg == 14 && R == 3 && S == 3 && gemm_x3_on() && gemm_x3_geom_ok(a) && ws_floats >= gemm_x3_ws_floats(Co, Kp)) return 16;
  return cfg;
}
DIAGAN_API int diagan_conv_gemm_set_splitk_fused(int mode) {
  DG_REQUIRE(mode >= -1 && mode <= 1, "set_splitk_fused: -1, 0 or 1");
  g_splitk_fused = mode;
  return DIAGAN_OK;
}
DIAGAN_API int diagan_conv_gemm_set_splitk_tickets(int* buf, int64_t slots) {
  DG_REQUIRE((buf && slots > 0) || (!buf && slots == 0), "set_splitk_tickets: a buffer with its slot count, or NULL and 0");
  g_tickets = buf;
  g_ticket_slots = (long)slots;
  return DIAGAN_OK;
}
struct diagan_conv_opts {
  int32_t wino, wino4, wino4x, gemm_x3, gemm_x3b, splitk_fused, force_ksplit, tune;
  int32_t* tickets;
  int64_t ticket_slots;
};
static_assert(sizeof(diagan_conv_opts) == 48, "diagan_conv_opts layout");
DIAGAN_API int diagan_conv_gemm_next_opts(const diagan_conv_opts* o) {
  if (!o) {
    g_opts_next = kNoOpts;
    return DIAGAN_OK;
  }
  DG_REQUIRE(o->wino >= -1 && o->wino <= 1 && o->wino4 >= -1 && o->wino4 <= 2 && o->wino4x >= -1 && o->wino4x <= 1 && o->gemm_x3 >= -1 &&
                 o->gemm_x3 <= 1 && o->gemm_x3b >= -1 && o->gemm_x3b <= 1 && o->splitk_fused >= -1 && o->splitk_fused <= 1 &&
                 o->force_ksplit >= 0 && o->tune >= -1,
             "conv_gemm_next_opts: a field out of range (-1 = process default; force_ksplit 0 = the launch policy)");
  DG_REQUIRE(!o->tickets || o->ticket_slots > 0, "conv_gemm_next_opts: a ticket buffer needs its slot count");
  g_opts_next = CallOpts{o->wino, o->wino4, o->wino4x, o->gemm_x3, o->gemm_x3b, o->splitk_fused, o->force_ksplit, o->tune, o->tickets,
                         (long)o->ticket_slots};
  return DIAGAN_OK;
}
DIAGAN_API int diagan_conv_gemm_pending_opts(diagan_conv_opts* o) {
  DG_REQUIRE(o, "conv_gemm_pending_opts: null");
  const CallOpts& c = g_opts_next;
  *o = diagan_conv_opts{c.wino, c.wino4, c.wino4x, c.gemm_x3, c.gemm_x3b, c.splitk_fused, c.force_ksplit, c.tune, c.tickets,
                        (int64_t)c.ticket_slots};
  return DIAGAN_OK;
}
DIAGAN_API int diagan_conv_gemm_last_cfg(void) { return g_last_cfg; }

DIAGAN_API int diagan_conv_gemm_set_stamp_buffer(unsigned long long* buf, int64_t slots) {
  g_stamps = buf;
  g_stamp_slots = buf ? (long)slots : 0;
  return DIAGAN_OK;
}
DIAGAN_API int diagan_conv_gemm_tune(int force_ksplit, int flags, int lds_delta_bytes) {
  g_force_ksplit = force_ksplit;
  g_tune_flags = flags;
  g_lds_delta = lds_delta_bytes;
  return DIAGAN_OK;
}
```

### self-diagnosing-gan_amd/csrc/conv_gemm_x3.hip

```cpp
#include "conv_common.h"
#include "wino_weights.h"
#include <stdlib.h>

namespace diagan {

constexpr int GX_ROW = 40;
constexpr int GX_PLANE = 64 * GX_ROW;
constexpr int GX_STAGE = 6 * GX_PLANE;
constexpr int GX_LDS_BYTES = 4 * GX_STAGE * 2;

typedef __bf16 gx_bf16x8 __attribute__((ext_vector_type(8)));
typedef unsigned gx_u32x4 __attribute__((ext_vector_type(4)));

__global__ __launch_bounds__(256) void gx3_weight_kernel(const float* __restrict__ w, unsigned short* __restrict__ wx, long quads) {
  const long plane = quads * 4;
  for (long i = (long)blockIdx.x * 256 + threadIdx.x; i < quads; i += (long)gridDim.x * 256) gx3_split_quad(w, wx, i, plane);
}

template <int PRO>
__global__ __launch_bounds__(512) void conv_gemm_x3_kernel(const ConvGemmArgs a, const unsigned short* __restrict__ wx) {
  extern __shared__ __attribute__((aligned(16))) unsigned short lds[];
  const ConvGeom& g = a.g;
  const int tid = threadIdx.x, lane = tid & 63, wave = __builtin_amdgcn_readfirstlane(tid >> 6);
  const int kg = wave >> 2, wg = wave & 3, wm = wg >> 1, wn = wg & 1;
  const int tg = tid & 255, lrow = tg >> 2, lq = tg & 3;
  const int tiles_n = (g.Co + 63) >> 6;
  const int tile = xcd_remap(blockIdx.x, gridDim.x);
  const int m0 = (tile / tiles_n) * 64, n0 = (tile % tiles_n) * 64;
  unsigned short* const stage0 = lds + kg * 2 * GX_STAGE;

  const int cpt = g.Ci >> 5;
  const int nk = g.R * g.S * cpt, kh = nk >> 1;
  const int k_begin = kg * kh, k_end = k_begin + kh;

  const int m = m0 + lrow;
  int oy = 0, ox = 0, pixbase = 0;
  const bool mv = m < a.M;
  {
    const unsigned t = fdiv((unsigned)(mv ? m : 0), a.dWo);
    ox = (mv ? m : 0) - (int)t * g.Wo;
    const unsigned b = fdiv(t, a.dHo);
    oy = (int)t - (int)b * g.Ho;
    pixbase = (((int)b * g.Hi + oy + g.off) * g.Wi + ox + g.off) * g.Ci * 4 + lq * 32;
  }
  const __amdgpu_buffer_rsrc_t xsrc = __builtin_amdgcn_make_buffer_rsrc(
      const_cast<float*>(a.x), 0, (int)((unsigned)g.B * g.Hi * g.Wi * g.Ci * 4u), 0x00020000);
  const long wplane = (long)g.Co * g.Kp;
  const __amdgpu_buffer_rsrc_t wsrc = __builtin_amdgcn_make_buffer_rsrc(
      const_cast<unsigned short*>(wx), 0, (int)((unsigned)(3 * wplane) * 2u), 0x00020000);
  const int n = n0 + lrow;
  const unsigned wrow = n < g.Co ? (unsigned)n * (unsigned)g.Kp * 2u + (unsigned)lq * 16u : 0x80000000u;
  const unsigned wpl = (unsigned)wplane * 2u;

  struct Staged { f32x4 a[2]; gx_u32x4 b[3]; };
  Staged sA, sB;
  auto load_step = [&](int kk, Staged& r) __attribute__((always_inline)) {
    const int tap = kk / cpt, c0 = (kk - tap * cpt) << 5;
    const int rr = tap / g.S, ss = tap - rr * g.S;
    const int iy = oy + g.off + rr * g.dr, ix = ox + g.off + ss * g.dr;
    const bool ok = mv && kk < k_end && (unsigned)iy < (unsigned)g.Hi && (unsigned)ix < (unsigned)g.Wi;
    const unsigned off = (unsigned)(pixbase + ((rr * g.Wi + ss) * g.dr * g.Ci + c0) * 4) | (ok ? 0u : 0x80000000u);
    r.a[0] = __builtin_bit_cast(f32x4, __builtin_amdgcn_raw_buffer_load_b128(xsrc, off, 0, 0));
    r.a[1] = __builtin_bit_cast(f32x4, __builtin_amdgcn_raw_buffer_load_b128(xsrc, off, 16, 0));
    const unsigned wo = (kk < k_end ? wrow : 0x80000000u) + (unsigned)kk * 64u;
#pragma unroll
    for (int p = 0; p < 3; ++p) r.b[p] = __builtin_bit_cast(gx_u32x4, __builtin_amdgcn_raw_buffer_load_b128(wsrc, wo + p * wpl, 0, 0));
  };
  const int sto = lrow * GX_ROW + lq * 8;
  auto store_step = [&](int buf, const Staged& r) __attribute__((always_inline)) {
    unsigned short* st = stage0 + buf * GX_STAGE;
    f32x4 v0 = r.a[0], v1 = r.a[1];
    if (PRO == PRO_RELU) {
#pragma unroll
      for (int e = 0; e < 4; ++e) { v0[e] = fmaxf(v0[e], 0.f); v1[e] = fmaxf(v1[e], 0.f); }
    }
    u32x2 a0, a1, a2, b0, b1, b2;
    x3_split(v0, a0, a1, a2);
    x3_split(v1, b0, b1, b2);
    *reinterpret_cast<gx_u32x4*>(st + sto) = gx_u32x4{a0[0], a0[1], b0[0], b0[1]};
    *reinterpret_cast<gx_u32x4*>(st + GX_PLANE + sto) = gx_u32x4{a1[0], a1[1], b1[0], b1[1]};
    *reinterpret_cast<gx_u32x4*>(st + 2 * GX_PLANE + sto) = gx_u32x4{a2[0], a2[1], b2[0], b2[1]};
#pragma unroll
    for (int p = 0; p < 3; ++p) *reinterpret_cast<gx_u32x4*>(st + (3 + p) * GX_PLANE + sto) = r.b[p];
  };

  f32x16 acc3[3];
#pragma unroll
  for (int p = 0; p < 3; ++p)
#pragma unroll
    for (int e = 0; e < 16; ++e) acc3[p][e] = 0.f;
  const int fi = lane & 31, fh = lane >> 5;
  const int fa = (wm * 32 + fi) * GX_ROW, fb = (wn * 32 + fi) * GX_ROW;
  const int oa01 = (fh ? GX_PLANE : 0) + fa, oa02 = (fh ? 2 * GX_PLANE : 0) + fa;
  const int ob00 = 3 * GX_PLANE + fb, ob11 = 4 * GX_PLANE + fb, ob20 = (fh ? 3 : 5) * GX_PLANE + fb;
  auto mfmas = [&](int buf) __attribute__((always_inline)) {
    const unsigned short* st = stage0 + buf * GX_STAGE;
#pragma unroll
    for (int c = 0; c < 4; ++c) {
      const gx_bf16x8 a01 = *reinterpret_cast<const gx_bf16x8*>(st + oa01 + c * 8);
      const gx_bf16x8 a02 = *reinterpret_cast<const gx_bf16x8*>(st + oa02 + c * 8);
      const gx_bf16x8 b00 = *reinterpret_cast<const gx_bf16x8*>(st + ob00 + c * 8);
      const gx_bf16x8 b11 = *reinterpret_cast<const gx_bf16x8*>(st + ob11 + c * 8);
      const gx_bf16x8 b20 = *reinterpret_cast<const gx_bf16x8*>(st + ob20 + c * 8);
      acc3[0] = __builtin_amdgcn_mfma_f32_32x32x16_bf16(a01, b00, acc3[0], 0, 0, 0);
      acc3[1] = __builtin_amdgcn_mfma_f32_32x32x16_bf16(a01, b11, acc3[1], 0, 0, 0);
      acc3[2] = __builtin_amdgcn_mfma_f32_32x32x16_bf16(a02, b20, acc3[2], 0, 0, 0);
    }
  };

  load_step(k_begin, sA);
  load_step(k_begin + 1, sB);
  store_step(0, sA);
  __syncthreads();
  for (int kk = k_begin; kk < k_end; kk += 2) {
    load_step(kk + 2, sA);
    mfmas(0);
    if (kk + 1 < k_end) store_step(1, sB);
    __syncthreads();
    if (kk + 1 >= k_end) break;
    load_step(kk + 3, sB);
    mfmas(1);
    if (kk + 2 < k_end) store_step(0, sA);
    __syncthreads();
  }
  f32x16 acc = acc3[0] + acc3[1] + acc3[2];

  float* xch = reinterpret_cast<float*>(lds);
  if (kg == 1) {
#pragma unroll
    for (int e = 0; e < 16; ++e) xch[e * 256 + tg] = acc[e];
  }
  __syncthreads();
  if (kg == 1) return;
#pragma unroll
  for (int e = 0; e < 16; ++e) acc[e] += xch[e * 256 + tg];

  const float sc0 = a.scale0 ? a.scale0[0] : a.out_scale, sc1 = a.scale1 ? a.scale1[0] : a.out_scale;
  const int split = a.scale0 ? a.scale_split : 0x7fffffff;
  const unsigned rowbytes = (unsigned)g.Co * 4u, ybytes = (unsigned)a.M * rowbytes;
  const __amdgpu_buffer_rsrc_t ysrc = __builtin_amdgcn_make_buffer_rsrc(a.y, 0, (int)ybytes, 0x00020000);
  const __amdgpu_buffer_rsrc_t rsrc = __builtin_amdgcn_make_buffer_rsrc(
      const_cast<float*>(a.residual ? a.residual : a.y), 0, a.residual ? (int)ybytes : 0, 0x00020000);
  const __amdgpu_buffer_rsrc_t msrc = __builtin_amdgcn_make_buffer_rsrc(
      const_cast<float*>(a.mask_src ? a.mask_src : a.y), 0, a.mask_src ? (int)ybytes : 0, 0x00020000);
  const float rfloor = a.res_relu ? 0.f : -__builtin_huge_valf();
  const int nc = n0 + wn * 32 + fi;
  const bool col_ok = nc < g.Co;
  const float bv = (a.bias && col_ok) ? a.bias[nc] : 0.f;
  const int mrow = m0 + wm * 32 + 4 * fh;
  const unsigned vbase = col_ok ? ((unsigned)mrow * g.Co + nc) * 4u : 0x80000000u;
  const bool hr = a.residual != nullptr, hm = a.mask_src != nullptr;
  float rres[16], rmsk[16];
  if (hr) {
#pragma unroll
    for (int e = 0; e < 16; ++e)
      rres[e] = __builtin_bit_cast(float, __builtin_amdgcn_raw_buffer_load_b32(rsrc, vbase, (int)(((e & 3) + 8 * (e >> 2)) * rowbytes), 0));
  }
  if (hm) {
#pragma unroll
    for (int e = 0; e < 16; ++e)
      rmsk[e] = __builtin_bit_cast(float, __builtin_amdgcn_raw_buffer_load_b32(msrc, vbase, (int)(((e & 3) + 8 * (e >> 2)) * rowbytes), 0));
  }
#pragma unroll
  for (int e = 0; e < 16; ++e) {
    const int k = (e & 3) + 8 * (e >> 2);
    float v = fmaf(acc[e], (mrow + k) < split ? sc0 : sc1, bv);
    if (hr) v += fmaxf(rres[e], rfloor);
    if (hm) v = rmsk[e] > 0.f ? v : v * a.mask_slope;
    __builtin_amdgcn_raw_buffer_store_b32(__float_as_uint(v), ysrc, vbase, (int)(k * rowbytes), 0);
  }
}

long gemm_x3_ws_floats(int Co, int Kp) { return ((long)Co * Kp * 3 + 1) / 2; }

bool gemm_x3_geom_ok(const ConvGemmArgs& a) {
  const ConvGeom& g = a.g;
  return g.sy == 1 && g.up == 1 && (g.Ci & 31) == 0 && g.Kp == g.R * g.S * g.Ci && ((g.R * g.S * (g.Ci >> 5)) & 1) == 0 &&
         (g.Co & 3) == 0 && (a.pro_mode == PRO_NONE || a.pro_mode == PRO_RELU) && !a.stat_partials && a.pro_group_rows == 0 &&
         !a.res_up && (long)g.Co * g.Kp * 6 < (1L << 31);
}

int launch_gemm_x3(const ConvGemmArgs& a, float* ws, hipStream_t st) {
  const ConvGeom& g = a.g;
  const long fl = gemm_x3_ws_floats(g.Co, g.Kp);
  const float* ready = wino_weights_ready(WK_GX3, 0, 1.f, fl);
  const unsigned short* wx = reinterpret_cast<const unsigned short*>(ready);
  if (!ready) {
    const long quads = (long)g.Co * g.Kp / 4;
    long blocks = (quads + 255) / 256;
    if (blocks > 2048) blocks = 2048;
    hipLaunchKernelGGL(gx3_weight_kernel, dim3((int)blocks), dim3(256), 0, st, a.w, reinterpret_cast<unsigned short*>(ws), quads);
    wx = reinterpret_cast<const unsigned short*>(ws);
  }
  const int tiles = cdiv(a.M, 64) * cdiv(g.Co, 64);
  static FuncAttrLatch latch_none, latch_relu;
  if (a.pro_mode == PRO_RELU) {
    DG_LDS(latch_relu, conv_gemm_x3_kernel<PRO_RELU>, GX_LDS_BYTES);
    hipLaunchKernelGGL(conv_gemm_x3_kernel<PRO_RELU>, dim3(tiles), dim3(512), GX_LDS_BYTES, st, a, wx);
  } else {
    DG_LDS(latch_none, conv_gemm_x3_kernel<PRO_NONE>, GX_LDS_BYTES);
    hipLaunchKernelGGL(conv_gemm_x3_kernel<PRO_NONE>, dim3(tiles), dim3(512), GX_LDS_BYTES, st, a, wx);
  }
  return check_launch("conv_gemm_x3");
}

}
```

### self-diagnosing-gan_amd/diagan/ops/conv.py

```python
import torch

from diagan import _native as nat

PRO_NONE, PRO_RELU, PRO_AFFINE_RELU, PRO_LRELU, PRO_AFFINE = 0, 1, 2, 3, 4
PRO_BOX, PRO_BOX_RELU = 5, 6
TILE_SHAPES = {1: (128, 128, 2, 2, 32, False), 2: (128, 64, 2, 2, 32, False), 3: (64, 64, 2, 2, 32, False),
               4: (128, 64, 4, 1, 32, False), 5: (256, 64, 4, 1, 32, False), 6: (64, 64, 2, 2, 64, False),
               7: (64, 64, 2, 2, 32, True), 8: (128, 64, 2, 2, 32, True), 14: (64, 64, 2, 2, 32, True)}


def gemm_kernel_name(cfg, mode, Co=128, w4pool=False, Ci=0, RS=9, mapped=False):
    if cfg in (11, 12) and w4pool:
        return f"conv_wino4_kernel<{mode if cfg == 11 else 0},{cfg - 10},false>"
    if cfg == 9:
        return f"conv_wino_kernel<{mode}>"
    if cfg in (13, 15):
        x3 = "true" if (nat.fn("diagan_conv_gemm_get_wino4x")() > 0 and Ci % 32 == 0) else "false"
        return f"conv_wino4_kernel<{mode},{0 if cfg == 13 else 3},{x3}>"
    if cfg == 11:
        return f"conv_wino_pool_kernel<{mode},false,{2 if Co % 128 == 0 else 1}>"
    if cfg == 12:
        return f"conv_wino_pool_kernel<0,true,{2 if Co % 128 == 0 else 1}>"
    if cfg == 17:
        return f"conv_gemm_x3b_kernel<{mode},{'true' if mapped else 'false'}>"
    if cfg == 16:
        return f"conv_gemm_x3_kernel<{mode}>"
    bm, bn, wm, wn, bk, fp = TILE_SHAPES[cfg]
    kg = ",2" if cfg == 14 else ",1"
    return f"conv_gemm_kernel<{bm},{bn},{wm},{wn},{bk},{mode},false,{'true' if fp else 'false'}{kg}>"


class KernelTimer:

    def __init__(self, only=None):
        self.records = []
        self.only = only

    def wants_any(self):
        return self.only is None or len(self.only) > 0

    def begin(self, name=None):
        if self.only is not None and name not in self.only:
            return None
        ev = torch.cuda.Event(enable_timing=True)
        ev.record()
        return ev

    def end(self, name, flop, start, shape=None):
        stop = torch.cuda.Event(enable_timing=True)
        stop.record()
        self.records.append((name, flop, start, stop, shape))

    def summary(self):
        out = {}
        for name, flop, s, e, _ in self.records:
            d = out.setdefault(name, dict(launches=0, flop=0.0, seconds=0.0))
            d['launches'] += 1
            d['flop'] += flop
            d['seconds'] += s.elapsed_time(e) * 1e-3
        return out

    def by_shape(self):
        out = {}
        for name, flop, s, e, shape in self.records:
            d = out.setdefault((name,) + tuple(shape or ()), dict(launches=0, flop=0.0, seconds=0.0))
            d['launches'] += 1
            d['flop'] += flop
            d['seconds'] += s.elapsed_time(e) * 1e-3
        return out


TIMER = None
_NAME_CACHE = {}


import ctypes as _ct
import os as _os

WINO_BATCH = _os.environ.get("DIAGAN_WINO_BATCH", "1") != "0"


class WinoWeights:
    __slots__ = ("w_of", "Co", "Ci", "Kp", "fmt", "u", "ready", "used")

    def __init__(self, w_of, Co, Ci, Kp):
        self.w_of, self.Co, self.Ci, self.Kp = w_of, Co, Ci, Kp
        self.fmt, self.u, self.ready, self.used = None, None, None, False


_LWF = (_ct.c_int(), _ct.c_int(), _ct.c_float(), _ct.c_int64(), _ct.c_int64())
_LWF_REFS = tuple(_ct.byref(v) for v in _LWF)


def last_weight_format():
    nat.fn("diagan_conv_gemm_last_weight_format")(*_LWF_REFS)
    k, f, sc, n, cnt = _LWF
    return (k.value, f.value, sc.value, n.value), cnt.value


class WinoWeightBatch:

    def __init__(self):
        self.sites = []
        self._table_key, self._tables = None, None

    def site(self, w_of, Co, Ci, Kp):
        s = WinoWeights(w_of, Co, Ci, Kp)
        self.sites.append(s)
        return s

    def prepare(self, version):
        if not WINO_BATCH:
            return
        import numpy as np
        todo = [s for s in self.sites if s.fmt is not None and s.fmt[0] and s.used and s.ready != version]
        if not todo:
            return
        key = tuple((id(s), s.fmt, s.w_of().data_ptr()) for s in todo)
        if key != self._table_key:
            desc = np.dtype([('w', np.uint64), ('u', np.uint64), ('i', np.int32, 6), ('scale', np.float32), ('pad', np.int32)])
            tab, blk = np.zeros(len(todo), dtype=desc), 0
            for j, s in enumerate(todo):
                w = s.w_of()
                if s.u is None or s.u.numel() != s.fmt[3] or s.u.device != w.device:
                    s.u = torch.empty(s.fmt[3], dtype=torch.float32, device=w.device)
                tab[j]['w'], tab[j]['u'] = w.data_ptr(), s.u.data_ptr()
                tab[j]['i'] = [s.Co, s.Ci, s.Kp, s.fmt[0], s.fmt[1], blk]
                tab[j]['scale'] = s.fmt[2]
                blk += nat.fn("diagan_wino_weight_blocks")(s.Co, s.Ci)
            dev_tab = torch.from_numpy(tab.view(np.uint8).copy()).to(todo[0].w_of().device)
            self._table_key, self._tables = key, (dev_tab, len(todo), blk)
        tab, n, blocks = self._tables
        nat.call("diagan_wino_weights_batched", nat.ptr(tab), n, blocks, nat.current_stream())
        for s in todo:
            s.ready = version


def _hint(wsite, version):
    if wsite is not None and WINO_BATCH and wsite.u is not None and wsite.ready == version and wsite.fmt is not None:
        nat.call("diagan_conv_gemm_weights_hint", wsite.u.data_ptr(), wsite.fmt[0], wsite.fmt[1], wsite.fmt[2])


def _learn(wsite):
    if wsite is not None and WINO_BATCH:
        fmt, _ = last_weight_format()
        wsite.used = True
        if fmt != wsite.fmt:
            wsite.fmt, wsite.ready = fmt, None


def set_winograd(mode):
    nat.call("diagan_conv_gemm_set_wino", -1 if mode is None else (1 if mode else 0))


def set_winograd4x(mode):
    nat.call("diagan_conv_gemm_set_wino4x", -1 if mode is None else (1 if mode else 0))


def set_winograd4(mode):
    nat.call("diagan_conv_gemm_set_wino4", -1 if mode is None else (2 if mode == 'force-pool' else (1 if mode else 0)))


def round_up(x, m):
    return (x + m - 1) // m * m


class Geom:

    def __init__(self, kind, Ci, Co, R, S, stride=1, pad=0):
        assert kind in ('conv', 'convT')
        self.kind, self.Ci, self.Co, self.R, self.S, self.stride, self.pad = kind, Ci, Co, R, S, stride, pad
        self.Kp = round_up(R * S * Ci, 32)
        self.Kd = round_up(R * S * Co, 32)

    def out_hw(self, Hi, Wi):
        if self.kind == 'conv':
            return ((Hi + 2 * self.pad - self.R) // self.stride + 1,
                    (Wi + 2 * self.pad - self.S) // self.stride + 1)
        return ((Hi - 1) * self.stride - 2 * self.pad + self.R, (Wi - 1) * self.stride - 2 * self.pad + self.S)

    def fwd_params(self):
        return (self.stride, 1, -self.pad, 1) if self.kind == 'conv' else (1, -1, self.pad, self.stride)

    def dgrad_params(self):
        return (1, -1, self.pad, self.stride) if self.kind == 'conv' else (self.stride, 1, -self.pad, 1)


def _pro3(pro):
    if pro is None:
        return PRO_NONE, None, None
    if len(pro) > 3 and pro[3]:
        raise RuntimeError("grouped BatchNorm prologues exist for the forward kernels only")
    return tuple(pro)[:3]


def set_gemm_x3(on):
    nat.call("diagan_conv_gemm_set_x3", -1 if on is None else (1 if on else 0))
    nat.call("diagan_conv_gemm_set_x3b", -1 if on is None else (1 if on else 0))


def set_gemm_x3b(on):
    nat.call("diagan_conv_gemm_set_x3b", -1 if on is None else (1 if on else 0))


def set_x3_pieces(n):
    nat.call("diagan_conv_gemm_set_x3_pieces", 0 if n is None else int(n))


def set_wgrad_x3(on):
    nat.call("diagan_conv_wgrad_set_x3", -1 if on is None else (int(on) if on else 0))


def wgrad_uses_x3(geom, B, Hi, Wi, Ho, Wo, mode=0, bias_off=-1):
    sy, dr, off, up = geom.fwd_params()
    return bool(nat.fn("diagan_conv_wgrad_uses_x3")(B, Hi, Wi, geom.Ci, Ho, Wo, geom.Co, geom.R, geom.S, sy, dr, off, up, geom.Kp,
                                                    mode, bias_off))


_TICKETS = {}


def set_splitk_fused(on):
    nat.call("diagan_conv_gemm_set_splitk_fused", -1 if on is None else (1 if on else 0))
    if on:
        dev = torch.cuda.current_device()
        if dev not in _TICKETS:
            _TICKETS[dev] = torch.zeros(1 << 16, dtype=torch.int32, device=torch.device('cuda', dev))
        nat.call("diagan_conv_gemm_set_splitk_tickets", _TICKETS[dev].data_ptr(), _TICKETS[dev].numel())
    else:
        nat.call("diagan_conv_gemm_set_splitk_tickets", None, 0)


class ConvOpts(_ct.Structure):
    _fields_ = [(n, _ct.c_int32) for n in ("wino", "wino4", "wino4x", "gemm_x3", "gemm_x3b", "splitk_fused", "force_ksplit", "tune")] + \
               [("tickets", _ct.c_void_p), ("ticket_slots", _ct.c_int64)]


def next_opts(tickets=None, **fields):
    o = ConvOpts(-1, -1, -1, -1, -1, -1, 0, -1, None, 0)
    for k, v in fields.items():
        setattr(o, k, int(v))
    if tickets is not None:
        o.tickets, o.ticket_slots = tickets.data_ptr(), tickets.numel()
    nat.call("diagan_conv_gemm_next_opts", _ct.byref(o))


def pending_opts():
    o = ConvOpts()
    nat.call("diagan_conv_gemm_pending_opts", _ct.byref(o))
    return o


def _opts_key(o):
    return tuple(getattr(o, n) for n, _ in ConvOpts._fields_[:8])


def _without_wino(o):
    m = ConvOpts.from_buffer_copy(o)
    m.wino, m.wino4 = 0, 0
    return m


def last_cfg():
    return nat.fn("diagan_conv_gemm_last_cfg")()


def wg_x_shape(x, pro):
    B, H, W, Ci = x.shape
    if pro is not None and int(pro[0]) >= PRO_BOX:
        return B, H + 1, W + 1, Ci
    return B, H, W, Ci


def _chk(t, name):
    if t is None:
        return
    if not (t.is_cuda and t.dtype == torch.float32 and t.is_contiguous()):
        raise RuntimeError(f"{name}: expected a contiguous CUDA float32 tensor, got "
                           f"{t.dtype} {t.device} contiguous={t.is_contiguous()}")


def _gemm(x, w, out, geo_params, R, S, Kp, bias, residual, mask_src, mask_slope, pro, out_scale, tile_cfg,
          res_relu=False, row_scale=None, want_stats=False, wino=True, res_up=False, pool=False, unpool=False, up_in=False,
          wsite=None, wversion=None, res_unpool=False, out_map=None):
    B, Hi, Wi, Ci = x.shape
    _, Ho, Wo, Co = out.shape
    if out_map is not None:
        Ho, Wo = out_map[9], out_map[10]
    if up_in:
        Hi, Wi, tile_cfg = 2 * Hi, 2 * Wi, 15
        if pool or unpool or mask_src is not None:
            raise RuntimeError("conv_gemm: the up-sampled-input launch takes no pooling and no backward mask")
    if unpool:
        Hi, Wi, tile_cfg = 2 * Hi, 2 * Wi, 12
    if pool:
        Ho, Wo, tile_cfg = 2 * Ho, 2 * Wo, 11
        if want_stats or res_up or mask_src is not None:
            raise RuntimeError("conv_gemm: the pooled launch takes no statistics, mask or half-resolution residual")
    mode, scale, shift, group_imgs = (tuple(pro) + (0,))[:4] if pro is not None else (PRO_NONE, None, None, 0)
    for t, n in ((x, 'x'), (w, 'w'), (out, 'out'), (bias, 'bias'), (residual, 'residual'),
                 (mask_src, 'mask_src'), (scale, 'pro_scale'), (shift, 'pro_shift')):
        _chk(t, n)
    if w.shape != (Co, Kp):
        raise RuntimeError(f"conv_gemm: packed weight shape {tuple(w.shape)} != ({Co}, {Kp})")
    for t, n in ((residual, 'residual'), (mask_src, 'mask_src')):
        want = (B, Ho // 2, Wo // 2, Co) if ((res_up or res_unpool) and n == 'residual') else tuple(out.shape)
        if t is not None and tuple(t.shape) != want:
            raise RuntimeError(f"conv_gemm: {n} shape {tuple(t.shape)} != {want}")
    if (res_up or res_unpool) and (residual is None or res_relu or not wino or (res_up and res_unpool)):
        raise RuntimeError("conv_gemm: res_up / res_unpool need a half-resolution residual, no ReLU on it, and the Winograd kernel")
    sy, dr, off, up = geo_params
    stats = None
    if (mask_src is None and row_scale is None and out_scale == 1.0 and not res_relu and tile_cfg == 0 and not res_unpool
            and not want_stats and nat.fn("diagan_conv3x3_co4_supported")(Ci, Co, R, S, sy, dr, off, up)):
        t0 = TIMER.begin("conv3x3_co4_kernel") if TIMER is not None else None
        nat.call("diagan_conv3x3_co4", nat.ptr(x), nat.ptr(w), nat.ptr(out), nat.ptr(bias), nat.ptr(residual),
                 nat.ptr(scale), nat.ptr(shift), mode, B, Hi, Wi, Ci, dr, off, Kp, group_imgs, nat.current_stream())
        if t0 is not None:
            TIMER.end("conv3x3_co4_kernel", 2.0 * B * Ho * Wo * Co * R * S * Ci, t0,
                      (B * Ho * Wo, Co, R * S * Ci, f"pro{mode}"))
        return out
    if (mode == PRO_NONE and residual is None and mask_src is None and not res_relu and tile_cfg == 0 and not want_stats
            and nat.fn("diagan_conv3x3_ci4_supported")(Ci, Co, R, S, sy, dr, off, up)):
        t0 = TIMER.begin("conv3x3_ci4_kernel") if TIMER is not None else None
        nat.call("diagan_conv3x3_ci4", nat.ptr(x), nat.ptr(w), nat.ptr(out), nat.ptr(bias), out_scale,
                 nat.ptr(row_scale[0]) if row_scale else None, nat.ptr(row_scale[1]) if row_scale else None,
                 (B // 2) * Ho * Wo if row_scale else 0, B, Hi, Wi, Co, Kp, nat.current_stream())
        if t0 is not None:
            TIMER.end("conv3x3_ci4_kernel", 2.0 * B * Ho * Wo * Co * R * S * Ci, t0, (B * Ho * Wo, Co, R * S * Ci, "pro0"))
        return out
    ws = _splitk_ws(x.device)
    if tile_cfg == 0 and not wino:
        if want_stats:
            tile_cfg = nat.fn("diagan_conv_gemm_pick_cfg")(B * Ho * Wo, Co, Kp, 0)
        else:
            nat.call("diagan_conv_gemm_next_opts", _ct.byref(_without_wino(pending_opts())))
    if want_stats:
        M = B * Ho * Wo
        cfg = tile_cfg or nat.fn("diagan_conv_gemm_pick_cfg_grouped")(B, Hi, Wi, Ci, Ho, Wo, Co, R, S, sy, dr, off, up, Kp, 0,
                                                                       ws.numel(), group_imgs * Ho * Wo)
        bm = nat.fn("diagan_conv_gemm_tile_rows")(cfg)
        tiles = (M + bm - 1) // bm
        stats = (torch.empty((tiles, 2, Co), dtype=torch.float32, device=x.device), tiles)
        tile_cfg = cfg
    kname = None
    if TIMER is not None and TIMER.wants_any():
        key = (tile_cfg, B, Hi, Wi, Ci, Ho, Wo, Co, R, S, sy, dr, off, up, Kp, mode, want_stats, group_imgs, out_map is not None,
               mask_src is None, row_scale is None, res_relu, res_up, res_unpool, _opts_key(pending_opts()))
        kname = _NAME_CACHE.get(key)
        modes = (nat.fn("diagan_conv_gemm_get_wino")(), nat.fn("diagan_conv_gemm_get_wino4x")(), nat.fn("diagan_conv_gemm_get_x3")(),
                 nat.fn("diagan_conv_gemm_get_x3b")())
        if kname is None or _NAME_CACHE.get('modes') != modes:
            if _NAME_CACHE.get('modes') != modes:
                _NAME_CACHE.clear()
                _NAME_CACHE['modes'] = modes
            allow = 0 if want_stats else 1
            plain = mask_src is None and row_scale is None and not res_relu and not res_up and not res_unpool
            kname = gemm_kernel_name(tile_cfg or nat.fn("diagan_conv_gemm_final_cfg")(
                B, Hi, Wi, Ci, Ho, Wo, Co, R, S, sy, dr, off, up, Kp, allow, ws.numel(), group_imgs * Ho * Wo, mode,
                1 if plain else 0, 1 if want_stats else 0), mode, Co,
                w4pool=tile_cfg in (11, 12) and bool(nat.fn("diagan_conv_wino4_pool_used")(B, Ho, Wo, Ci, Co, ws.numel())), Ci=Ci, RS=R * S,
                mapped=out_map is not None)
            _NAME_CACHE[key] = kname
    t0 = TIMER.begin(kname) if TIMER is not None else None
    _hint(wsite, wversion)
    if out_map is not None:
        nat.call("diagan_conv_gemm_out_map", *out_map[:9])
    nat.call("diagan_conv_gemm", nat.ptr(x), nat.ptr(w), nat.ptr(out), nat.ptr(bias), nat.ptr(residual),
             (1 if res_relu else 0) | (2 if res_up else 0) | (4 if res_unpool else 0), nat.ptr(mask_src), mask_slope, nat.ptr(scale), nat.ptr(shift), mode, out_scale,
             nat.ptr(row_scale[0]) if row_scale else None, nat.ptr(row_scale[1]) if row_scale else None,
             (B // 2) * Ho * Wo if row_scale else 0,
             B, Hi, Wi, Ci, Ho, Wo, Co, R, S, sy, dr, off, up, Kp, tile_cfg, nat.ptr(ws), ws.numel(),
             nat.ptr(stats[0]) if stats else None, group_imgs * Ho * Wo, nat.current_stream())
    _learn(wsite)
    if t0 is not None:
        TIMER.end(kname, 2.0 * B * Ho * Wo * Co * R * S * Ci, t0,
                  (B * Ho * Wo, Co, R * S * Ci, f"pro{mode}{'+res' if residual is not None else ''}"
                                               f"{'+mask' if mask_src is not None else ''}{'+up' if up > 1 else ''}"))
    return (out, stats) if want_stats else out


_skws = {}


def _splitk_ws(dev):
    w = _skws.get(dev.index)
    if w is None:
        w = torch.empty(64 << 20, dtype=torch.float32, device=dev)
        _skws[dev.index] = w
    return w


def res_up_fused(geom, B, Hi, Wi, want_stats=False, group_imgs=0):
    Ho, Wo = geom.out_hw(Hi, Wi)
    sy, dr, off, up = geom.fwd_params()
    ws = _splitk_ws(torch.device('cuda', torch.cuda.current_device()))
    return nat.fn("diagan_conv_gemm_pick_cfg_grouped")(B, Hi, Wi, geom.Ci, Ho, Wo, geom.Co, geom.R, geom.S, sy, dr, off,
                                                       up, geom.Kp, 0 if want_stats else 1, ws.numel(),
                                                       group_imgs * Ho * Wo) in (9, 13)


def upin_fused(geom, B, Hl, Wl, group_imgs=0):
    Hi, Wi = 2 * Hl, 2 * Wl
    Ho, Wo = geom.out_hw(Hi, Wi)
    sy, dr, off, up = geom.fwd_params()
    ws = _splitk_ws(torch.device('cuda', torch.cuda.current_device()))
    return bool(nat.fn("diagan_conv_wino4_upin_supported")(B, Hi, Wi, geom.Ci, Ho, Wo, geom.Co, geom.R, geom.S, sy, dr, off, up,
                                                           ws.numel(), group_imgs * Ho * Wo))


def pool_fused(geom, B, Hi, Wi, pro=None):
    Ho, Wo = geom.out_hw(Hi, Wi)
    sy, dr, off, up = geom.fwd_params()
    mode = pro[0] if pro is not None else PRO_NONE
    ws = _splitk_ws(torch.device('cuda', torch.cuda.current_device()))
    return bool(nat.fn("diagan_conv_wino_pool_supported")(B, Hi, Wi, geom.Ci, Ho, Wo, geom.Co, geom.R, geom.S, sy, dr, off, up,
                                                          mode, ws.numel()))


def conv_fwd(geom, x, wf, bias=None, residual=None, pro=None, out=None, tile_cfg=0, res_relu=False, row_scale=None,
             want_stats=False, out_scale=1.0, wino=True, res_up=False, pool=False, up_in=False, wsite=None, wversion=None,
             out_map=None):
    B, Hi, Wi, Ci = x.shape
    if Ci != geom.Ci:
        raise RuntimeError(f"conv_fwd: input has {Ci} channels, layer expects {geom.Ci}")
    Ho, Wo = geom.out_hw(2 * Hi, 2 * Wi) if up_in else geom.out_hw(Hi, Wi)
    if pool:
        Ho, Wo = Ho // 2, Wo // 2
    if out_map is not None:
        if out is None:
            raise RuntimeError("conv_fwd: an output map needs the target tensor")
        out_map = tuple(out_map) + (out.shape[1], out.shape[2], Ho, Wo)
    if out is None:
        out = torch.empty((B, Ho, Wo, geom.Co), dtype=torch.float32, device=x.device)
    return _gemm(x, wf, out, geom.fwd_params(), geom.R, geom.S, geom.Kp, bias, residual, None, 0.0, pro, out_scale,
                 tile_cfg, res_relu=res_relu, row_scale=row_scale, want_stats=want_stats, wino=wino, res_up=res_up, pool=pool,
                 up_in=up_in, wsite=wsite, wversion=wversion, out_map=out_map)


def out_map_ok(geom, B, Hi, Wi, pro=None, wino=True):
    Ho, Wo = geom.out_hw(Hi, Wi)
    sy, dr, off, up = geom.fwd_params()
    ws = _splitk_ws(torch.device('cuda', torch.cuda.current_device()))
    mode = pro[0] if pro is not None else PRO_NONE
    pend = None if wino else pending_opts()
    if pend is not None:
        nat.call("diagan_conv_gemm_next_opts", _ct.byref(_without_wino(pend)))
    try:
        return nat.fn("diagan_conv_gemm_final_cfg")(B, Hi, Wi, geom.Ci, Ho, Wo, geom.Co, geom.R, geom.S, sy, dr, off, up, geom.Kp, 1,
                                                   ws.numel(), 0, mode, 1, 0) == 17
    finally:
        if pend is not None:
            nat.call("diagan_conv_gemm_next_opts", _ct.byref(pend))


def conv_dgrad(geom, dy, wd, in_hw, residual=None, mask_src=None, mask_slope=0.0, out=None, tile_cfg=0,
               row_scale=None, wino=True, unpool=False, wsite=None, wversion=None, res_unpool=False):
    B, Ho, Wo, Co = dy.shape
    if Co != geom.Co:
        raise RuntimeError(f"conv_dgrad: dy has {Co} channels, layer has {geom.Co}")
    Hi, Wi = in_hw
    if unpool and (2 * Ho, 2 * Wo) != tuple(geom.out_hw(Hi, Wi)):
        raise RuntimeError(f"conv_dgrad: pooled gradient {Ho}x{Wo} does not match the layer's output {geom.out_hw(Hi, Wi)}")
    if out is None:
        out = torch.empty((B, Hi, Wi, geom.Ci), dtype=torch.float32, device=dy.device)
    return _gemm(dy, wd, out, geom.dgrad_params(), geom.R, geom.S, geom.Kd, None, residual, mask_src, mask_slope,
                 None, 1.0, tile_cfg, row_scale=row_scale, wino=wino, unpool=unpool, wsite=wsite, wversion=wversion,
                 res_unpool=res_unpool)


def res_unpool_fused(geom, B, Hi, Wi):
    if Hi % 2 or Wi % 2 or _os.environ.get("DIAGAN_RES_UNPOOL", "1") == "0":
        return False
    Ho, Wo = geom.out_hw(Hi, Wi)
    sy, dr, off, up = geom.dgrad_params()
    ws = _splitk_ws(torch.device('cuda', torch.cuda.current_device()))
    return nat.fn("diagan_conv_gemm_pick_cfg_geom")(B, Ho, Wo, geom.Co, Hi, Wi, geom.Ci, geom.R, geom.S, sy, dr, off, up, geom.Kd, 1,
                                                    ws.numel()) in (9, 13)


def unpool_fused(geom, B, Hi, Wi):
    Ho, Wo = geom.out_hw(Hi, Wi)
    sy, dr, off, up = geom.dgrad_params()
    ws = _splitk_ws(torch.device('cuda', torch.cuda.current_device()))
    return bool(nat.fn("diagan_conv_wino_unpool_supported")(B, Ho, Wo, geom.Co, Hi, Wi, geom.Ci, geom.R, geom.S, sy, dr, off, up,
                                                            ws.numel()))


_slabs = {}
_slabs_retired = []


def _slab(dev, nfloat):
    key = (dev.index, )
    s = _slabs.get(key)
    if s is None or s.numel() < nfloat:
        if s is not None:
            _slabs_retired.append(s)
        s = torch.empty(max(nfloat, 1 << 22), dtype=torch.float32, device=dev)
        _slabs[key] = s
    return s


def conv_wgrad(geom, dy, x, grad, accumulate, pro=None, sn=None):
    B, Ho, Wo, Co = dy.shape
    _, Hi, Wi, Ci = wg_x_shape(x, pro)
    mode, scale, shift = _pro3(pro)
    for t, n in ((dy, 'dy'), (x, 'x'), (grad, 'grad'), (scale, 'pro_scale'), (shift, 'pro_shift')):
        _chk(t, n)
    M = B * Ho * Wo
    splits = wgrad_splits_geom(geom, B, Hi, Wi, Ho, Wo)
    n_elem = Co * geom.Kp
    extra = n_elem if sn is not None else 0
    slab = _slab(dy.device, splits * n_elem + extra)
    sy, dr, off, up = geom.fwd_params()
    st = nat.current_stream()
    timed = TIMER is not None and TIMER.wants_any()
    kn = _wgrad_kernel_name(Co, geom.Kp, mode, Ho, Wo, wino=wgrad_uses_wino(geom, Hi, Wi, Ho, Wo),
                            x3=wgrad_uses_x3(geom, B, Hi, Wi, Ho, Wo, mode, -1)) if timed else None
    t0 = TIMER.begin(kn) if timed else None
    nat.call("diagan_conv_wgrad", nat.ptr(dy), nat.ptr(x), nat.ptr(slab), splits, 1, n_elem, -1, nat.ptr(scale), nat.ptr(shift),
             mode, B, Hi, Wi, Ci, Ho, Wo, Co, geom.R, geom.S, sy, dr, off, up, geom.Kp, st)
    if t0 is not None:
        TIMER.end(kn, 2.0 * M * Co * geom.R * geom.S * Ci, t0,
                  (M, Co, geom.R * geom.S * Ci, f"pro{mode} x{splits}"))
    if sn is None:
        nat.call("diagan_wgrad_reduce", nat.ptr(slab), splits, n_elem, nat.ptr(grad), 1 if accumulate else 0,
                 None, None, st)
    else:
        W, u, v, state = sn
        G = slab[splits * n_elem: splits * n_elem + n_elem]
        nparts = (n_elem // 4 + 255) // 256
        parts = torch.empty(nparts, dtype=torch.float64, device=dy.device)
        nat.call("diagan_wgrad_reduce", nat.ptr(slab), splits, n_elem, G.data_ptr(), 0, nat.ptr(W),
                 nat.ptr(parts), st)
        nat.call("diagan_sn_grad_fix", G.data_ptr(), nat.ptr(parts), nparts, nat.ptr(u), nat.ptr(v),
                 nat.ptr(state), nat.ptr(grad), Co, geom.Kp, 1 if accumulate else 0, st)
    return grad


def wgrad_splits(M, Co, Kp):
    return nat.fn("diagan_conv_wgrad_splits")(M, Co, Kp)


def wgrad_splits_geom(geom, B, Hi, Wi, Ho, Wo):
    sy, dr, off, up = geom.fwd_params()
    return nat.fn("diagan_conv_wgrad_splits_geom")(B, Hi, Wi, geom.Ci, Ho, Wo, geom.Co, geom.R, geom.S, sy, dr, off, up,
                                                   geom.Kp)


def wgrad_uses_wino(geom, Hi, Wi, Ho, Wo):
    sy, dr, off, up = geom.fwd_params()
    return bool(nat.fn("diagan_conv_wgrad_uses_wino")(Hi, Wi, geom.Ci, Ho, Wo, geom.Co, geom.R, geom.S, sy, dr, off, up,
                                                      geom.Kp))


def small_co_wgrad(geom):
    sy, dr, off, up = geom.fwd_params()
    return bool(nat.fn("diagan_conv3x3_co4_wgrad_supported")(geom.Ci, geom.Co, geom.R, geom.S, sy, dr, off, up)
                and geom.Kp == 9 * geom.Ci)


def small_co_wgrad_splits(B, H):
    return nat.fn("diagan_conv3x3_co4_wgrad_splits")(B, H)


def conv_wgrad_into(geom, dy, x, slab, splits, stride, bias_off, pro=None, segments=1, pooled=False):
    B, Ho, Wo, Co = dy.shape
    _, Hi, Wi, Ci = wg_x_shape(x, pro)
    mode, scale, shift = _pro3(pro)
    sy, dr, off, up = geom.fwd_params()
    if segments == 1 and small_co_wgrad(geom):
        if splits != small_co_wgrad_splits(B, Ho):
            raise RuntimeError(f"conv_wgrad_into: slab has {splits} splits, the 4-channel kernel writes "
                               f"{small_co_wgrad_splits(B, Ho)}")
        t0 = TIMER.begin("conv3x3_co4_wgrad_kernel") if TIMER is not None else None
        nat.call("diagan_conv3x3_co4_wgrad", nat.ptr(dy), nat.ptr(x), nat.ptr(slab), stride, bias_off, nat.ptr(scale),
                 nat.ptr(shift), mode, B, Hi, Wi, Ci, geom.Kp, nat.current_stream())
        if t0 is not None:
            TIMER.end("conv3x3_co4_wgrad_kernel", 2.0 * B * Ho * Wo * Co * 9 * Ci, t0, (B * Ho * Wo, Co, 9 * Ci, f"pro{mode}"))
        return
    timed = TIMER is not None and TIMER.wants_any()
    kn = _wgrad_kernel_name(Co, geom.Kp, mode, Ho, Wo, wino=wgrad_uses_wino(geom, Hi, Wi, Ho, Wo),
                            x3=wgrad_uses_x3(geom, B, Hi, Wi, Ho, Wo, mode, bias_off)) if timed else None
    if kn is not None and pooled:
        kn += POOLED_TAG
    t0 = TIMER.begin(kn) if timed else None
    nat.call("diagan_conv_wgrad", nat.ptr(dy), nat.ptr(x), nat.ptr(slab), splits, segments, stride, bias_off, nat.ptr(scale),
             nat.ptr(shift), mode, B, Hi, Wi, Ci, Ho, Wo, Co, geom.R, geom.S, sy, dr, off, up, geom.Kp,
             nat.current_stream())
    if t0 is not None:
        px = B * Ho * Wo * (4 if pooled else 1)
        TIMER.end(kn, 2.0 * px * Co * geom.R * geom.S * Ci, t0, (px, Co, geom.R * geom.S * Ci, f"pro{mode}"))


WGRAD_BATCH = _os.environ.get("DIAGAN_WGRAD_BATCH", "1") != "0"
WGRAD_BATCH_MIN_STEPS = int(_os.environ.get("DIAGAN_WGRAD_BATCH_MIN_STEPS", str(1 << 30)))
_WG_JOB = None


def batched_wgrad_splits(jobs, slots=256, fixed=8.0):
    def plan(per):
        out, total, longest = [], 0, 0
        for tiles, steps, seg in jobs:
            seg_steps = -(-steps // seg)
            k = max(1, min(-(-seg_steps // per), max(1, seg_steps // 4)))
            out.append(k * seg)
            total += (tiles * k * seg + 7) // 8 * 8
            longest = max(longest, -(-seg_steps // k))
        return (-(-total // slots)) * (longest + fixed), out
    best, per = None, 4.0
    top = max(-(-steps // seg) for _, steps, seg in jobs)
    while True:
        cost, out = plan(int(per))
        if best is None or cost < best[0]:
            best = (cost, out)
        if per > top:
            return best[1]
        per = max(per + 1, per * 1.08)


_WG_TABS = {}


def conv_wgrad_batched(jobs, key=None, kernel_name=None, flop_scale=1.0, cache=None):
    global _WG_JOB
    import numpy as np
    if _WG_JOB is None:
        _WG_JOB = np.dtype([('p', np.uint64, 5), ('l', np.int64, 2), ('i', np.int32, 18)])
        assert _WG_JOB.itemsize == 128
    tabs = cache if cache is not None else _WG_TABS
    if key is not None and cache is None:
        key = (key,) + tuple((g.kind, g.Ci, g.Co, g.R, g.S, g.stride, g.pad, g.Kp, tuple(dy.shape), tuple(x.shape), sp, st, bo,
                              _pro3(pro)[0], seg) for g, dy, x, _, sp, st, bo, pro, seg in jobs)
    cached = tabs.get(key) if key is not None else None
    if cached is None:
        tab = np.zeros(len(jobs), dtype=_WG_JOB)
        flop, px, mode0 = 0.0, 0, None
        for j, (geom, dy, x, slab, splits, stride, bias_off, pro, segments) in enumerate(jobs):
            B, Ho, Wo, Co = dy.shape
            _, Hi, Wi, Ci = wg_x_shape(x, pro)
            mode = _pro3(pro)[0]
            mode0 = mode if mode0 is None else mode0
            sy, dr, off, up = geom.fwd_params()
            tab[j]['l'] = [stride, bias_off]
            tab[j]['i'] = [splits, segments, mode, B, Hi, Wi, Ci, Ho, Wo, Co, geom.R, geom.S, sy, dr, off, up, geom.Kp, 0]
            flop += 2.0 * B * Ho * Wo * Co * geom.R * geom.S * Ci
            px += B * Ho * Wo
        cached = (tab, flop, px, mode0)
        if key is not None:
            if len(tabs) > 256:
                tabs.clear()
            tabs[key] = cached
    tab, flop, px, mode0 = cached
    ptrs = []
    for geom, dy, x, slab, splits, stride, bias_off, pro, segments in jobs:
        scale, shift = (pro[1], pro[2]) if pro is not None and len(pro) > 2 else (None, None)
        ptrs.append((dy.data_ptr(), x.data_ptr(), slab.data_ptr(), 0 if scale is None else scale.data_ptr(),
                     0 if shift is None else shift.data_ptr()))
    tab['p'] = ptrs
    timed = TIMER is not None and TIMER.wants_any()
    kn = (kernel_name or f"conv_wgrad_wino_batched_kernel<{mode0}>") if timed else None
    t0 = TIMER.begin(kn) if timed else None
    nat.call("diagan_conv_wgrad_batched", tab.ctypes.data, len(jobs), nat.current_stream())
    if t0 is not None:
        g0 = jobs[0][0]
        TIMER.end(kn, flop * flop_scale, t0, (int(px * flop_scale), g0.Co, g0.R * g0.S * g0.Ci, f"pro{mode0} {len(jobs)} layers"))


def wgrad_batch_max():
    return nat.fn("diagan_conv_wgrad_batch_max")()


def wgrad_batch_class(geom, Hi, Wi, Ho, Wo, mode):
    sy, dr, off, up = geom.fwd_params()
    return nat.fn("diagan_conv_wgrad_batch_class")(Hi, Wi, geom.Ci, Ho, Wo, geom.Co, geom.R, geom.S, sy, dr, off, up, geom.Kp, mode)


def wgrad_batch_shape(geom, B, Ho, Wo, cls):
    if cls < 1000:
        return ((geom.Co + 63) // 64) * ((geom.Ci + 63) // 64), (B * (Ho // 2) * (Wo // 2) + 7) // 8, 256, 8.0
    bn, bk = (64 if geom.Co <= 64 else 128), (64 if geom.Kp <= 64 else 128)
    if bn == 128 and bk == 64:
        bn = 64
    slots = _WG_SLOTS64 if (bn == 64 and bk == 64) else 512
    return ((geom.Co + bn - 1) // bn) * ((geom.Kp + bk - 1) // bk), (B * Ho * Wo + 31) // 32, slots, 6.0


_WG_SLOTS64 = int(_os.environ.get("DIAGAN_WGRAD_SLOTS64", "512"))
POOLED_TAG = " [pooled gradient]"


def _wgrad_kernel_name(Co, Kp, mode=0, Ho=0, Wo=0, wino=False, x3=False):
    if wino:
        return f"conv_wgrad_wino_kernel<{mode}>"
    if x3:
        return "conv_wgrad_x3_kernel"
    bn, bk = (64 if Co <= 64 else 128), (64 if Kp <= 64 else 128)
    if bn == 128 and bk == 64:
        bn = 64
    if bk != 128:
        return f"conv_wgrad_kernel<{bn},{bk},-1,false>"
    p2 = Ho > 0 and Wo > 0 and (Ho & (Ho - 1)) == 0 and (Wo & (Wo - 1)) == 0
    return f"conv_wgrad_kernel<{bn},128,{mode},{'true' if p2 else 'false'}>"


def sn_power_iter(W, u_buffer, sigma_buffer, training=True, eps=1e-12):
    Co, Kp = W.shape
    dev = W.device
    u = torch.empty(Co, dtype=torch.float32, device=dev)
    v = torch.empty(Kp, dtype=torch.float32, device=dev)
    state = torch.empty(2, dtype=torch.float32, device=dev)
    work = torch.empty(Kp + Co, dtype=torch.float32, device=dev)
    nat.call("diagan_sn_power_iter", nat.ptr(W), nat.ptr(u_buffer), nat.ptr(sigma_buffer), nat.ptr(u), nat.ptr(v),
             nat.ptr(state), nat.ptr(work), Co, Kp, eps, 1 if training else 0, nat.current_stream())
    return u, v, state


def pack_weights(W, Co, Ci, RS, Kp, Kd, inv_sigma=None, Wf=None, Wd=None):
    nat.call("diagan_pack_weights", nat.ptr(W), nat.ptr(inv_sigma), nat.ptr(Wf), nat.ptr(Wd), Co, Ci, RS, Kp, Kd,
             nat.current_stream())



def pack_oihw(w_oihw, Kp, ci_pad=None):
    Co, Ci, R, S = w_oihw.shape
    Cp = ci_pad or Ci
    w = w_oihw.permute(0, 2, 3, 1)
    if Cp != Ci:
        w = torch.nn.functional.pad(w, (0, Cp - Ci))
    w = w.reshape(Co, R * S * Cp)
    out = torch.zeros((Co, Kp), dtype=w.dtype, device=w.device)
    out[:, : R * S * Cp] = w
    return out


def unpack_oihw(wp, Co, Ci, R, S, ci_pad=None):
    Cp = ci_pad or Ci
    w = wp[:, : R * S * Cp].reshape(Co, R, S, Cp)[..., :Ci]
    return w.permute(0, 3, 1, 2).contiguous()


def pack_iohw(w_iohw, Kp):
    return pack_oihw(w_iohw.permute(1, 0, 2, 3), Kp)


def unpack_iohw(wp, Ci, Co, R, S):
    return unpack_oihw(wp, Co, Ci, R, S).permute(1, 0, 2, 3).contiguous()
```

Measured before the change: 5233.

## Add LDS-resident halo form of the x3 bf16-split conv GEMM for 8x8 maps

Adds a resident variant of the three-way bf16-split 3x3 conv GEMM kernel for 8x8 spatial maps. The whole 10x10 input halo for a 64-pixel tile is loaded into LDS once and split into bf16 planes there, and each tap then reads the A operand from that halo. Only the weights still stream through double-buffered stages. This removes the per-tap re-reads of the input from global memory and the repeated split work. In exchange it needs more LDS, which can lower occupancy. It is on by default through an env switch and a new per-call option field, which also changes the size of the ABI struct.

```diff
diff --git a/include/diagan_conv_x3.h b/include/diagan_conv_x3.h
--- /dev/null
+++ b/include/diagan_conv_x3.h
@@ -0,0 +1,19 @@
+#ifndef DIAGAN_CONV_X3_H
+#define DIAGAN_CONV_X3_H
+
+#include <stdint.h>
+
+#ifdef __cplusplus
+extern "C" {
+#endif
+
+int diagan_conv_gemm_set_x3_resident(int mode);
+int diagan_conv_gemm_get_x3_resident(void);
+int diagan_conv_gemm_last_x3_form(void);
+int diagan_conv_gemm_x3_resident_ok(int B, int Hi, int Wi, int Ci, int Ho, int Wo, int Co, int R, int S, int sy, int dr, int off, int up,
+                                    int Kp, int pro_mode);
+
+#ifdef __cplusplus
+}
+#endif
+#endif
diff --git a/include/diagan_hip.h b/include/diagan_hip.h
--- a/include/diagan_hip.h
+++ b/include/diagan_hip.h
@@ -74,6 +74,7 @@
   int32_t wino, wino4, wino4x, gemm_x3, gemm_x3b, splitk_fused, force_ksplit, tune;
   int32_t* tickets;
   int64_t ticket_slots;
+  int32_t gemm_x3_resident;
 } diagan_conv_opts;
 int diagan_conv_gemm_next_opts(const diagan_conv_opts* opts);
 int diagan_conv_gemm_pending_opts(diagan_conv_opts* opts);
diff --git a/self-diagnosing-gan_amd/csrc/conv_gemm.hip b/self-diagnosing-gan_amd/csrc/conv_gemm.hip
--- a/self-diagnosing-gan_amd/csrc/conv_gemm.hip
+++ b/self-diagnosing-gan_amd/csrc/conv_gemm.hip
@@ -16,8 +16,9 @@
                                           int off, int up);
 
 namespace diagan {
-int launch_gemm_x3(const ConvGemmArgs& a, float* ws, hipStream_t st);
+int launch_gemm_x3(const ConvGemmArgs& a, float* ws, bool resident, hipStream_t st);
 bool gemm_x3_geom_ok(const ConvGemmArgs& a);
+bool gemm_x3_resident_ok(const ConvGemmArgs& a);
 long gemm_x3_ws_floats(int Co, int Kp);
 int launch_gemm_x3b(const ConvGemmArgs& a, const OutMap& map, float* ws, hipStream_t st);
 bool gemm_x3b_geom_ok(const ConvGemmArgs& a);
@@ -619,21 +620,26 @@
 
 static int g_gemm_x3 = -1;
 static int g_gemm_x3b = -1;
+static int g_gemm_x3_resident = -1;
+static Switch kGemmX3Resident{{"DIAGAN_GEMM_X3_RESIDENT", 1}};
 static int x3b_min_tiles() { return kGemmX3bMinTiles.env(); }
 static thread_local OutMap g_map_next = {0, 0, 0, 0, 0, 0, 0, 0, 0};
 struct CallOpts {
   int wino, wino4, wino4x, gemm_x3, gemm_x3b, splitk_fused, force_ksplit, tune;
   int* tickets;
   long ticket_slots;
+  int gemm_x3_resident;
 };
-static const CallOpts kNoOpts = {-1, -1, -1, -1, -1, -1, 0, -1, nullptr, 0};
+static const CallOpts kNoOpts = {-1, -1, -1, -1, -1, -1, 0, -1, nullptr, 0, -1};
 static thread_local CallOpts g_opts_next = kNoOpts, g_opts_now = kNoOpts;
 static thread_local int g_last_cfg = 0;
+static thread_local int g_last_x3_form = 0;
 int call_opt_wino4x() { return g_opts_now.wino4x; }
 static int sel_wino() { return kWino.get(g_opts_now.wino, g_wino); }
 static int sel_wino4() { return g_opts_now.wino4 >= 0 ? g_opts_now.wino4 : g_wino4; }
 static int sel_force_ksplit() { return g_opts_now.force_ksplit > 0 ? g_opts_now.force_ksplit : g_force_ksplit; }
 static bool gemm_x3_on() { return kGemmX3.get(g_opts_now.gemm_x3, g_gemm_x3) != 0; }
+static bool gemm_x3_resident_on() { return kGemmX3Resident.get(g_opts_now.gemm_x3_resident, g_gemm_x3_resident) != 0; }
 static bool gemm_x3b_on() { return kGemmX3b.get(g_opts_now.gemm_x3b, g_gemm_x3b) != 0; }
 static bool x3b_takes(const ConvGemmArgs& a, int cfg, int64_t ws_floats) {
   if (!gemm_x3b_on() || !(cfg == 1 || cfg == 3 || cfg == 5 || cfg == 7 || cfg == 8)) return false;
@@ -944,7 +950,9 @@
                "32-channel K-steps, Kp == R*S*Ci, prologue none / ReLU, no statistics, and %ld floats of workspace", gemm_x3_ws_floats(Co, Kp));
     a.ksplit = 1;
     g_last_cfg = 16;
-    return launch_gemm_x3(a, splitk_ws, st);
+    const bool resident = gemm_x3_resident_on() && gemm_x3_resident_ok(a);
+    g_last_x3_form = resident ? 2 : 1;
+    return launch_gemm_x3(a, splitk_ws, resident, st);
   }
   if (cfg == 17) {
     DG_REQUIRE(gemm_x3b_geom_ok(a) && splitk_ws && gemm_x3b_ws_floats(Co, Kp) <= splitk_ws_floats,
@@ -1074,6 +1082,21 @@
   return DIAGAN_OK;
 }
 DIAGAN_API int diagan_conv_gemm_get_x3b(void) { return gemm_x3b_on() ? 1 : 0; }
+DIAGAN_API int diagan_conv_gemm_set_x3_resident(int mode) {
+  DG_REQUIRE(mode >= -1 && mode <= 1, "set_x3_resident: -1, 0 or 1");
+  g_gemm_x3_resident = mode;
+  return DIAGAN_OK;
+}
+DIAGAN_API int diagan_conv_gemm_get_x3_resident(void) { return gemm_x3_resident_on() ? 1 : 0; }
+DIAGAN_API int diagan_conv_gemm_last_x3_form(void) { return g_last_x3_form; }
+DIAGAN_API int diagan_conv_gemm_x3_resident_ok(int B, int Hi, int Wi, int Ci, int Ho, int Wo, int Co, int R, int S, int sy, int dr, int off,
+                                               int up, int Kp, int pro_mode) {
+  ConvGemmArgs a = {};
+  a.pro_mode = pro_mode;
+  a.M = B * Ho * Wo;
+  a.g = ConvGeom{B, Hi, Wi, Ci, Ho, Wo, Co, R, S, sy, dr, off, up, R * S * Ci, Kp};
+  return gemm_x3_resident_ok(a) ? 1 : 0;
+}
 namespace diagan { void x3_set_pieces(int n); int x3_pieces(); }
 DIAGAN_API int diagan_conv_gemm_set_x3_pieces(int n) {
   diagan::x3_set_pieces(n);
@@ -1127,8 +1150,9 @@
   int32_t wino, wino4, wino4x, gemm_x3, gemm_x3b, splitk_fused, force_ksplit, tune;
   int32_t* tickets;
   int64_t ticket_slots;
+  int32_t gemm_x3_resident;
 };
-static_assert(sizeof(diagan_conv_opts) == 48, "diagan_conv_opts layout");
+static_assert(sizeof(diagan_conv_opts) == 56, "diagan_conv_opts layout");
 DIAGAN_API int diagan_conv_gemm_next_opts(const diagan_conv_opts* o) {
   if (!o) {
     g_opts_next = kNoOpts;
@@ -1136,18 +1160,18 @@
   }
   DG_REQUIRE(o->wino >= -1 && o->wino <= 1 && o->wino4 >= -1 && o->wino4 <= 2 && o->wino4x >= -1 && o->wino4x <= 1 && o->gemm_x3 >= -1 &&
                  o->gemm_x3 <= 1 && o->gemm_x3b >= -1 && o->gemm_x3b <= 1 && o->splitk_fused >= -1 && o->splitk_fused <= 1 &&
-                 o->force_ksplit >= 0 && o->tune >= -1,
+                 o->force_ksplit >= 0 && o->tune >= -1 && o->gemm_x3_resident >= -1 && o->gemm_x3_resident <= 1,
              "conv_gemm_next_opts: a field out of range (-1 = process default; force_ksplit 0 = the launch policy)");
   DG_REQUIRE(!o->tickets || o->ticket_slots > 0, "conv_gemm_next_opts: a ticket buffer needs its slot count");
   g_opts_next = CallOpts{o->wino, o->wino4, o->wino4x, o->gemm_x3, o->gemm_x3b, o->splitk_fused, o->force_ksplit, o->tune, o->tickets,
-                         (long)o->ticket_slots};
+                         (long)o->ticket_slots, o->gemm_x3_resident};
   return DIAGAN_OK;
 }
 DIAGAN_API int diagan_conv_gemm_pending_opts(diagan_conv_opts* o) {
   DG_REQUIRE(o, "conv_gemm_pending_opts: null");
   const CallOpts& c = g_opts_next;
   *o = diagan_conv_opts{c.wino, c.wino4, c.wino4x, c.gemm_x3, c.gemm_x3b, c.splitk_fused, c.force_ksplit, c.tune, c.tickets,
-                        (int64_t)c.ticket_slots};
+                        (int64_t)c.ticket_slots, c.gemm_x3_resident};
   return DIAGAN_OK;
 }
 DIAGAN_API int diagan_conv_gemm_last_cfg(void) { return g_last_cfg; }
diff --git a/self-diagnosing-gan_amd/csrc/conv_gemm_x3.hip b/self-diagnosing-gan_amd/csrc/conv_gemm_x3.hip
--- a/self-diagnosing-gan_amd/csrc/conv_gemm_x3.hip
+++ b/self-diagnosing-gan_amd/csrc/conv_gemm_x3.hip
@@ -1,4 +1,5 @@
 #include "conv_common.h"
+#include "gemm_x3_halo.h"
 #include "wino_weights.h"
 #include <stdlib.h>
 
@@ -9,6 +10,8 @@
 constexpr int GX_STAGE = 6 * GX_PLANE;
 constexpr int GX_LDS_BYTES = 4 * GX_STAGE * 2;
 
+static_assert(GXR_WSTAGE == 3 * GX_PLANE, "a weight stage of the resident form: the B half of GX_STAGE");
+
 typedef __bf16 gx_bf16x8 __attribute__((ext_vector_type(8)));
 typedef unsigned gx_u32x4 __attribute__((ext_vector_type(4)));
 
@@ -17,112 +20,9 @@
   for (long i = (long)blockIdx.x * 256 + threadIdx.x; i < quads; i += (long)gridDim.x * 256) gx3_split_quad(w, wx, i, plane);
 }
 
-template <int PRO>
-__global__ __launch_bounds__(512) void conv_gemm_x3_kernel(const ConvGemmArgs a, const unsigned short* __restrict__ wx) {
-  extern __shared__ __attribute__((aligned(16))) unsigned short lds[];
-  const ConvGeom& g = a.g;
-  const int tid = threadIdx.x, lane = tid & 63, wave = __builtin_amdgcn_readfirstlane(tid >> 6);
-  const int kg = wave >> 2, wg = wave & 3, wm = wg >> 1, wn = wg & 1;
-  const int tg = tid & 255, lrow = tg >> 2, lq = tg & 3;
-  const int tiles_n = (g.Co + 63) >> 6;
-  const int tile = xcd_remap(blockIdx.x, gridDim.x);
-  const int m0 = (tile / tiles_n) * 64, n0 = (tile % tiles_n) * 64;
-  unsigned short* const stage0 = lds + kg * 2 * GX_STAGE;
-
-  const int cpt = g.Ci >> 5;
-  const int nk = g.R * g.S * cpt, kh = nk >> 1;
-  const int k_begin = kg * kh, k_end = k_begin + kh;
-
-  const int m = m0 + lrow;
-  int oy = 0, ox = 0, pixbase = 0;
-  const bool mv = m < a.M;
-  {
-    const unsigned t = fdiv((unsigned)(mv ? m : 0), a.dWo);
-    ox = (mv ? m : 0) - (int)t * g.Wo;
-    const unsigned b = fdiv(t, a.dHo);
-    oy = (int)t - (int)b * g.Ho;
-    pixbase = (((int)b * g.Hi + oy + g.off) * g.Wi + ox + g.off) * g.Ci * 4 + lq * 32;
-  }
-  const __amdgpu_buffer_rsrc_t xsrc = __builtin_amdgcn_make_buffer_rsrc(
-      const_cast<float*>(a.x), 0, (int)((unsigned)g.B * g.Hi * g.Wi * g.Ci * 4u), 0x00020000);
-  const long wplane = (long)g.Co * g.Kp;
-  const __amdgpu_buffer_rsrc_t wsrc = __builtin_amdgcn_make_buffer_rsrc(
-      const_cast<unsigned short*>(wx), 0, (int)((unsigned)(3 * wplane) * 2u), 0x00020000);
-  const int n = n0 + lrow;
-  const unsigned wrow = n < g.Co ? (unsigned)n * (unsigned)g.Kp * 2u + (unsigned)lq * 16u : 0x80000000u;
-  const unsigned wpl = (unsigned)wplane * 2u;
-
-  struct Staged { f32x4 a[2]; gx_u32x4 b[3]; };
-  Staged sA, sB;
-  auto load_step = [&](int kk, Staged& r) __attribute__((always_inline)) {
-    const int tap = kk / cpt, c0 = (kk - tap * cpt) << 5;
-    const int rr = tap / g.S, ss = tap - rr * g.S;
-    const int iy = oy + g.off + rr * g.dr, ix = ox + g.off + ss * g.dr;
-    const bool ok = mv && kk < k_end && (unsigned)iy < (unsigned)g.Hi && (unsigned)ix < (unsigned)g.Wi;
-    const unsigned off = (unsigned)(pixbase + ((rr * g.Wi + ss) * g.dr * g.Ci + c0) * 4) | (ok ? 0u : 0x80000000u);
-    r.a[0] = __builtin_bit_cast(f32x4, __builtin_amdgcn_raw_buffer_load_b128(xsrc, off, 0, 0));
-    r.a[1] = __builtin_bit_cast(f32x4, __builtin_amdgcn_raw_buffer_load_b128(xsrc, off, 16, 0));
-    const unsigned wo = (kk < k_end ? wrow : 0x80000000u) + (unsigned)kk * 64u;
-#pragma unroll
-    for (int p = 0; p < 3; ++p) r.b[p] = __builtin_bit_cast(gx_u32x4, __builtin_amdgcn_raw_buffer_load_b128(wsrc, wo + p * wpl, 0, 0));
-  };
-  const int sto = lrow * GX_ROW + lq * 8;
-  auto store_step = [&](int buf, const Staged& r) __attribute__((always_inline)) {
-    unsigned short* st = stage0 + buf * GX_STAGE;
-    f32x4 v0 = r.a[0], v1 = r.a[1];
-    if (PRO == PRO_RELU) {
-#pragma unroll
-      for (int e = 0; e < 4; ++e) { v0[e] = fmaxf(v0[e], 0.f); v1[e] = fmaxf(v1[e], 0.f); }
-    }
-    u32x2 a0, a1, a2, b0, b1, b2;
-    x3_split(v0, a0, a1, a2);
-    x3_split(v1, b0, b1, b2);
-    *reinterpret_cast<gx_u32x4*>(st + sto) = gx_u32x4{a0[0], a0[1], b0[0], b0[1]};
-    *reinterpret_cast<gx_u32x4*>(st + GX_PLANE + sto) = gx_u32x4{a1[0], a1[1], b1[0], b1[1]};
-    *reinterpret_cast<gx_u32x4*>(st + 2 * GX_PLANE + sto) = gx_u32x4{a2[0], a2[1], b2[0], b2[1]};
-#pragma unroll
-    for (int p = 0; p < 3; ++p) *reinterpret_cast<gx_u32x4*>(st + (3 + p) * GX_PLANE + sto) = r.b[p];
-  };
-
-  f32x16 acc3[3];
-#pragma unroll
-  for (int p = 0; p < 3; ++p)
-#pragma unroll
-    for (int e = 0; e < 16; ++e) acc3[p][e] = 0.f;
-  const int fi = lane & 31, fh = lane >> 5;
-  const int fa = (wm * 32 + fi) * GX_ROW, fb = (wn * 32 + fi) * GX_ROW;
-  const int oa01 = (fh ? GX_PLANE : 0) + fa, oa02 = (fh ? 2 * GX_PLANE : 0) + fa;
-  const int ob00 = 3 * GX_PLANE + fb, ob11 = 4 * GX_PLANE + fb, ob20 = (fh ? 3 : 5) * GX_PLANE + fb;
-  auto mfmas = [&](int buf) __attribute__((always_inline)) {
-    const unsigned short* st = stage0 + buf * GX_STAGE;
-#pragma unroll
-    for (int c = 0; c < 4; ++c) {
-      const gx_bf16x8 a01 = *reinterpret_cast<const gx_bf16x8*>(st + oa01 + c * 8);
-      const gx_bf16x8 a02 = *reinterpret_cast<const gx_bf16x8*>(st + oa02 + c * 8);
-      const gx_bf16x8 b00 = *reinterpret_cast<const gx_bf16x8*>(st + ob00 + c * 8);
-      const gx_bf16x8 b11 = *reinterpret_cast<const gx_bf16x8*>(st + ob11 + c * 8);
-      const gx_bf16x8 b20 = *reinterpret_cast<const gx_bf16x8*>(st + ob20 + c * 8);
-      acc3[0] = __builtin_amdgcn_mfma_f32_32x32x16_bf16(a01, b00, acc3[0], 0, 0, 0);
-      acc3[1] = __builtin_amdgcn_mfma_f32_32x32x16_bf16(a01, b11, acc3[1], 0, 0, 0);
-      acc3[2] = __builtin_amdgcn_mfma_f32_32x32x16_bf16(a02, b20, acc3[2], 0, 0, 0);
-    }
-  };
-
-  load_step(k_begin, sA);
-  load_step(k_begin + 1, sB);
-  store_step(0, sA);
-  __syncthreads();
-  for (int kk = k_begin; kk < k_end; kk += 2) {
-    load_step(kk + 2, sA);
-    mfmas(0);
-    if (kk + 1 < k_end) store_step(1, sB);
-    __syncthreads();
-    if (kk + 1 >= k_end) break;
-    load_step(kk + 3, sB);
-    mfmas(1);
-    if (kk + 2 < k_end) store_step(0, sA);
-    __syncthreads();
-  }
+__device__ __forceinline__ void gx3_finish(const ConvGemmArgs& a, const f32x16 (&acc3)[3], unsigned short* lds, int kg, int tg, int m0, int n0,
+                                           int wm, int wn, int fi, int fh) {
+  const ConvGeom& g = a.g;
   f32x16 acc = acc3[0] + acc3[1] + acc3[2];
 
   float* xch = reinterpret_cast<float*>(lds);
@@ -171,6 +71,248 @@
   }
 }
 
+template <int PRO>
+__global__ __launch_bounds__(512) void conv_gemm_x3_kernel(const ConvGemmArgs a, const unsigned short* __restrict__ wx) {
+  extern __shared__ __attribute__((aligned(16))) unsigned short lds[];
+  const ConvGeom& g = a.g;
+  const int tid = threadIdx.x, lane = tid & 63, wave = __builtin_amdgcn_readfirstlane(tid >> 6);
+  const int kg = wave >> 2, wg = wave & 3, wm = wg >> 1, wn = wg & 1;
+  const int tg = tid & 255, lrow = tg >> 2, lq = tg & 3;
+  const int tiles_n = (g.Co + 63) >> 6;
+  const int tile = xcd_remap(blockIdx.x, gridDim.x);
+  const int m0 = (tile / tiles_n) * 64, n0 = (tile % tiles_n) * 64;
+  unsigned short* const stage0 = lds + kg * 2 * GX_STAGE;
+
+  const int cpt = g.Ci >> 5;
+  const int nk = g.R * g.S * cpt, kh = nk >> 1;
+  const int k_begin = kg * kh, k_end = k_begin + kh;
+
+  const int m = m0 + lrow;
+  int oy = 0, ox = 0, pixbase = 0;
+  const bool mv = m < a.M;
+  {
+    const unsigned t = fdiv((unsigned)(mv ? m : 0), a.dWo);
+    ox = (mv ? m : 0) - (int)t * g.Wo;
+    const unsigned b = fdiv(t, a.dHo);
+    oy = (int)t - (int)b * g.Ho;
+    pixbase = (((int)b * g.Hi + oy + g.off) * g.Wi + ox + g.off) * g.Ci * 4 + lq * 32;
+  }
+  const __amdgpu_buffer_rsrc_t xsrc = __builtin_amdgcn_make_buffer_rsrc(
+      const_cast<float*>(a.x), 0, (int)((unsigned)g.B * g.Hi * g.Wi * g.Ci * 4u), 0x00020000);
+  const long wplane = (long)g.Co * g.Kp;
+  const __amdgpu_buffer_rsrc_t wsrc = __builtin_amdgcn_make_buffer_rsrc(
+      const_cast<unsigned short*>(wx), 0, (int)((unsigned)(3 * wplane) * 2u), 0x00020000);
+  const int n = n0 + lrow;
+  const unsigned wrow = n < g.Co ? (unsigned)n * (unsigned)g.Kp * 2u + (unsigned)lq * 16u : 0x80000000u;
+  const unsigned wpl = (unsigned)wplane * 2u;
+
+  struct Staged { f32x4 a[2]; gx_u32x4 b[3]; };
+  Staged sA, sB;
+  auto load_step = [&](int kk, Staged& r) __attribute__((always_inline)) {
+    const int tap = kk / cpt, c0 = (kk - tap * cpt) << 5;
+    const int rr = tap / g.S, ss = tap - rr * g.S;
+    const int iy = oy + g.off + rr * g.dr, ix = ox + g.off + ss * g.dr;
+    const bool ok = mv && kk < k_end && (unsigned)iy < (unsigned)g.Hi && (unsigned)ix < (unsigned)g.Wi;
+    const unsigned off = (unsigned)(pixbase + ((rr * g.Wi + ss) * g.dr * g.Ci + c0) * 4) | (ok ? 0u : 0x80000000u);
+    r.a[0] = __builtin_bit_cast(f32x4, __builtin_amdgcn_raw_buffer_load_b128(xsrc, off, 0, 0));
+    r.a[1] = __builtin_bit_cast(f32x4, __builtin_amdgcn_raw_buffer_load_b128(xsrc, off, 16, 0));
+    const unsigned wo = (kk < k_end ? wrow : 0x80000000u) + (unsigned)kk * 64u;
+#pragma unroll
+    for (int p = 0; p < 3; ++p) r.b[p] = __builtin_bit_cast(gx_u32x4, __builtin_amdgcn_raw_buffer_load_b128(wsrc, wo + p * wpl, 0, 0));
+  };
+  const int sto = lrow * GX_ROW + lq * 8;
+  auto store_step = [&](int buf, const Staged& r) __attribute__((always_inline)) {
+    unsigned short* st = stage0 + buf * GX_STAGE;
+    f32x4 v0 = r.a[0], v1 = r.a[1];
+    if (PRO == PRO_RELU) {
+#pragma unroll
+      for (int e = 0; e < 4; ++e) { v0[e] = fmaxf(v0[e], 0.f); v1[e] = fmaxf(v1[e], 0.f); }
+    }
+    u32x2 a0, a1, a2, b0, b1, b2;
+    x3_split(v0, a0, a1, a2);
+    x3_split(v1, b0, b1, b2);
+    *reinterpret_cast<gx_u32x4*>(st + sto) = gx_u32x4{a0[0], a0[1], b0[0], b0[1]};
+    *reinterpret_cast<gx_u32x4*>(st + GX_PLANE + sto) = gx_u32x4{a1[0], a1[1], b1[0], b1[1]};
+    *reinterpret_cast<gx_u32x4*>(st + 2 * GX_PLANE + sto) = gx_u32x4{a2[0], a2[1], b2[0], b2[1]};
+#pragma unroll
+    for (int p = 0; p < 3; ++p) *reinterpret_cast<gx_u32x4*>(st + (3 + p) * GX_PLANE + sto) = r.b[p];
+  };
+
+  f32x16 acc3[3];
+#pragma unroll
+  for (int p = 0; p < 3; ++p)
+#pragma unroll
+    for (int e = 0; e < 16; ++e) acc3[p][e] = 0.f;
+  const int fi = lane & 31, fh = lane >> 5;
+  const int fa = (wm * 32 + fi) * GX_ROW, fb = (wn * 32 + fi) * GX_ROW;
+  const int oa01 = (fh ? GX_PLANE : 0) + fa, oa02 = (fh ? 2 * GX_PLANE : 0) + fa;
+  const int ob00 = 3 * GX_PLANE + fb, ob11 = 4 * GX_PLANE + fb, ob20 = (fh ? 3 : 5) * GX_PLANE + fb;
+  auto mfmas = [&](int buf) __attribute__((always_inline)) {
+    const unsigned short* st = stage0 + buf * GX_STAGE;
+#pragma unroll
+    for (int c = 0; c < 4; ++c) {
+      const gx_bf16x8 a01 = *reinterpret_cast<const gx_bf16x8*>(st + oa01 + c * 8);
+      const gx_bf16x8 a02 = *reinterpret_cast<const gx_bf16x8*>(st + oa02 + c * 8);
+      const gx_bf16x8 b00 = *reinterpret_cast<const gx_bf16x8*>(st + ob00 + c * 8);
+      const gx_bf16x8 b11 = *reinterpret_cast<const gx_bf16x8*>(st + ob11 + c * 8);
+      const gx_bf16x8 b20 = *reinterpret_cast<const gx_bf16x8*>(st + ob20 + c * 8);
+      acc3[0] = __builtin_amdgcn_mfma_f32_32x32x16_bf16(a01, b00, acc3[0], 0, 0, 0);
+      acc3[1] = __builtin_amdgcn_mfma_f32_32x32x16_bf16(a01, b11, acc3[1], 0, 0, 0);
+      acc3[2] = __builtin_amdgcn_mfma_f32_32x32x16_bf16(a02, b20, acc3[2], 0, 0, 0);
+    }
+  };
+
+  load_step(k_begin, sA);
+  load_step(k_begin + 1, sB);
+  store_step(0, sA);
+  __syncthreads();
+  for (int kk = k_begin; kk < k_end; kk += 2) {
+    load_step(kk + 2, sA);
+    mfmas(0);
+    if (kk + 1 < k_end) store_step(1, sB);
+    __syncthreads();
+    if (kk + 1 >= k_end) break;
+    load_step(kk + 3, sB);
+    mfmas(1);
+    if (kk + 2 < k_end) store_step(0, sA);
+    __syncthreads();
+  }
+  gx3_finish(a, acc3, lds, kg, tg, m0, n0, wm, wn, fi, fh);
+}
+
+template <int PRO>
+__global__ __launch_bounds__(512) void conv_gemm_x3_kernel_resident(const ConvGemmArgs a, const unsigned short* __restrict__ wx) {
+  extern __shared__ __attribute__((aligned(16))) unsigned short lds[];
+  const ConvGeom& g = a.g;
+  const int tid = threadIdx.x, lane = tid & 63, wave = __builtin_amdgcn_readfirstlane(tid >> 6);
+  const int kg = wave >> 2, wg = wave & 3, wm = wg >> 1, wn = wg & 1;
+  const int tg = tid & 255, lrow = tg >> 2, lq = tg & 3;
+  const int tiles_n = (g.Co + 63) >> 6;
+  const int tile = xcd_remap(blockIdx.x, gridDim.x);
+  const int m0 = (tile / tiles_n) * 64, n0 = (tile % tiles_n) * 64;
+  unsigned short* const stage0 = lds + kg * 2 * GXR_WSTAGE;
+  unsigned short* const halo = lds + 4 * GXR_WSTAGE;
+  const int hpix = gxr_pix_pitch(g.Ci), hrow = gxr_row_pitch(g.Ci), hplane = GXR_HALO * hrow;
+
+  const int cpt = g.Ci >> 5;
+  const int nk = 9 * cpt, kh = nk >> 1;
+  const int k_begin = kg * kh, k_end = k_begin + kh;
+
+  const long wplane = (long)g.Co * g.Kp;
+  const __amdgpu_buffer_rsrc_t wsrc = __builtin_amdgcn_make_buffer_rsrc(
+      const_cast<unsigned short*>(wx), 0, (int)((unsigned)(3 * wplane) * 2u), 0x00020000);
+  const int n = n0 + lrow;
+  const unsigned wrow = n < g.Co ? (unsigned)n * (unsigned)g.Kp * 2u + (unsigned)lq * 16u : 0x80000000u;
+  const unsigned wpl = (unsigned)wplane * 2u;
+
+  struct Staged { gx_u32x4 b[3]; };
+  Staged sA, sB;
+  auto load_step = [&](int kk, Staged& r) __attribute__((always_inline)) {
+    const unsigned wo = (kk < k_end ? wrow : 0x80000000u) + (unsigned)kk * 64u;
+#pragma unroll
+    for (int p = 0; p < 3; ++p) r.b[p] = __builtin_bit_cast(gx_u32x4, __builtin_amdgcn_raw_buffer_load_b128(wsrc, wo + p * wpl, 0, 0));
+  };
+  const int sto = lrow * GX_ROW + lq * 8;
+  auto store_step = [&](int buf, const Staged& r) __attribute__((always_inline)) {
+    unsigned short* st = stage0 + buf * GXR_WSTAGE;
+#pragma unroll
+    for (int p = 0; p < 3; ++p) *reinterpret_cast<gx_u32x4*>(st + p * GX_PLANE + sto) = r.b[p];
+  };
+  load_step(k_begin, sA);
+  load_step(k_begin + 1, sB);
+
+  {
+    const int cq = g.Ci >> 3;
+    const gx_u32x4 zero = {0u, 0u, 0u, 0u};
+    for (int i = tid; i < GXR_BORDER * cq; i += 512) {
+      const int bp = i / cq, ch = i - bp * cq;
+      int hy, hx;
+      gxr_border_pixel(bp, hy, hx);
+      unsigned short* d = halo + hy * hrow + hx * hpix + ch * 8;
+#pragma unroll
+      for (int p = 0; p < 3; ++p) *reinterpret_cast<gx_u32x4*>(d + p * hplane) = zero;
+    }
+    const __amdgpu_buffer_rsrc_t xsrc = __builtin_amdgcn_make_buffer_rsrc(
+        const_cast<float*>(a.x), 0, (int)((unsigned)g.B * 64u * g.Ci * 4u), 0x00020000);
+    const int chunks = 64 * cq;
+    for (int i0 = tid; i0 < chunks; i0 += 1024) {
+      f32x4 v[2][2];
+      int dst[2];
+#pragma unroll
+      for (int j = 0; j < 2; ++j) {
+        const int i = i0 + j * 512;
+        const int pix = i / cq, ch = i - pix * cq, m = m0 + pix;
+        const unsigned off = (((unsigned)m * g.Ci + ch * 8) * 4u) | ((i < chunks && m < a.M) ? 0u : 0x80000000u);
+        v[j][0] = __builtin_bit_cast(f32x4, __builtin_amdgcn_raw_buffer_load_b128(xsrc, off, 0, 0));
+        v[j][1] = __builtin_bit_cast(f32x4, __builtin_amdgcn_raw_buffer_load_b128(xsrc, off, 16, 0));
+        dst[j] = i < chunks ? ((pix >> 3) + 1) * hrow + ((pix & 7) + 1) * hpix + ch * 8 : -1;
+      }
+#pragma unroll
+      for (int j = 0; j < 2; ++j) {
+        if (dst[j] < 0) continue;
+        f32x4 v0 = v[j][0], v1 = v[j][1];
+        if (PRO == PRO_RELU) {
+#pragma unroll
+          for (int e = 0; e < 4; ++e) { v0[e] = fmaxf(v0[e], 0.f); v1[e] = fmaxf(v1[e], 0.f); }
+        }
+        u32x2 a0, a1, a2, b0, b1, b2;
+        x3_split(v0, a0, a1, a2);
+        x3_split(v1, b0, b1, b2);
+        unsigned short* d = halo + dst[j];
+        *reinterpret_cast<gx_u32x4*>(d) = gx_u32x4{a0[0], a0[1], b0[0], b0[1]};
+        *reinterpret_cast<gx_u32x4*>(d + hplane) = gx_u32x4{a1[0], a1[1], b1[0], b1[1]};
+        *reinterpret_cast<gx_u32x4*>(d + 2 * hplane) = gx_u32x4{a2[0], a2[1], b2[0], b2[1]};
+      }
+    }
+  }
+
+  f32x16 acc3[3];
+#pragma unroll
+  for (int p = 0; p < 3; ++p)
+#pragma unroll
+    for (int e = 0; e < 16; ++e) acc3[p][e] = 0.f;
+  const int fi = lane & 31, fh = lane >> 5;
+  const int fa = gxr_halo_off(wm * 32 + fi, 0, 0, 1, -1, g.Ci), fb = (wn * 32 + fi) * GX_ROW;
+  const int oa01 = (fh ? hplane : 0) + fa, oa02 = (fh ? 2 * hplane : 0) + fa;
+  const int ob00 = fb, ob11 = GX_PLANE + fb, ob20 = (fh ? 0 : 2) * GX_PLANE + fb;
+  int rr = (k_begin / cpt) / 3, ss = k_begin / cpt - rr * 3, c0 = (k_begin - (k_begin / cpt) * cpt) << 5;
+  auto mfmas = [&](int buf) __attribute__((always_inline)) {
+    const unsigned short* st = stage0 + buf * GXR_WSTAGE;
+    const unsigned short* ha = halo + (1 + g.off + rr * g.dr) * hrow + (1 + g.off + ss * g.dr) * hpix + c0;
+#pragma unroll
+    for (int c = 0; c < 4; ++c) {
+      const gx_bf16x8 a01 = *reinterpret_cast<const gx_bf16x8*>(ha + oa01 + c * 8);
+      const gx_bf16x8 a02 = *reinterpret_cast<const gx_bf16x8*>(ha + oa02 + c * 8);
+      const gx_bf16x8 b00 = *reinterpret_cast<const gx_bf16x8*>(st + ob00 + c * 8);
+      const gx_bf16x8 b11 = *reinterpret_cast<const gx_bf16x8*>(st + ob11 + c * 8);
+      const gx_bf16x8 b20 = *reinterpret_cast<const gx_bf16x8*>(st + ob20 + c * 8);
+      acc3[0] = __builtin_amdgcn_mfma_f32_32x32x16_bf16(a01, b00, acc3[0], 0, 0, 0);
+      acc3[1] = __builtin_amdgcn_mfma_f32_32x32x16_bf16(a01, b11, acc3[1], 0, 0, 0);
+      acc3[2] = __builtin_amdgcn_mfma_f32_32x32x16_bf16(a02, b20, acc3[2], 0, 0, 0);
+    }
+    c0 += 32;
+    if (c0 == g.Ci) {
+      c0 = 0;
+      if (++ss == 3) { ss = 0; ++rr; }
+    }
+  };
+
+  store_step(0, sA);
+  __syncthreads();
+  for (int kk = k_begin; kk < k_end; kk += 2) {
+    load_step(kk + 2, sA);
+    mfmas(0);
+    if (kk + 1 < k_end) store_step(1, sB);
+    __syncthreads();
+    if (kk + 1 >= k_end) break;
+    load_step(kk + 3, sB);
+    mfmas(1);
+    if (kk + 2 < k_end) store_step(0, sA);
+    __syncthreads();
+  }
+  gx3_finish(a, acc3, lds, kg, tg, m0, n0, wm, wn, fi, fh);
+}
+
 long gemm_x3_ws_floats(int Co, int Kp) { return ((long)Co * Kp * 3 + 1) / 2; }
 
 bool gemm_x3_geom_ok(const ConvGemmArgs& a) {
@@ -180,7 +322,12 @@
          !a.res_up && (long)g.Co * g.Kp * 6 < (1L << 31);
 }
 
-int launch_gemm_x3(const ConvGemmArgs& a, float* ws, hipStream_t st) {
+bool gemm_x3_resident_ok(const ConvGemmArgs& a) {
+  const ConvGeom& g = a.g;
+  return gemm_x3_geom_ok(a) && gxr_shape_ok(g.B, g.Hi, g.Wi, g.Ci, g.Ho, g.Wo, g.R, g.S, g.dr, g.off);
+}
+
+int launch_gemm_x3(const ConvGemmArgs& a, float* ws, bool resident, hipStream_t st) {
   const ConvGeom& g = a.g;
   const long fl = gemm_x3_ws_floats(g.Co, g.Kp);
   const float* ready = wino_weights_ready(WK_GX3, 0, 1.f, fl);
@@ -193,8 +340,17 @@
     wx = reinterpret_cast<const unsigned short*>(ws);
   }
   const int tiles = cdiv(a.M, 64) * cdiv(g.Co, 64);
-  static FuncAttrLatch latch_none, latch_relu;
-  if (a.pro_mode == PRO_RELU) {
+  static FuncAttrLatch latch_none, latch_relu, latch_res_none, latch_res_relu;
+  if (resident) {
+    const size_t bytes = (size_t)gxr_lds_bytes(g.Ci);
+    if (a.pro_mode == PRO_RELU) {
+      DG_LDS(latch_res_relu, conv_gemm_x3_kernel_resident<PRO_RELU>, bytes);
+      hipLaunchKernelGGL(conv_gemm_x3_kernel_resident<PRO_RELU>, dim3(tiles), dim3(512), bytes, st, a, wx);
+    } else {
+      DG_LDS(latch_res_none, conv_gemm_x3_kernel_resident<PRO_NONE>, bytes);
+      hipLaunchKernelGGL(conv_gemm_x3_kernel_resident<PRO_NONE>, dim3(tiles), dim3(512), bytes, st, a, wx);
+    }
+  } else if (a.pro_mode == PRO_RELU) {
     DG_LDS(latch_relu, conv_gemm_x3_kernel<PRO_RELU>, GX_LDS_BYTES);
     hipLaunchKernelGGL(conv_gemm_x3_kernel<PRO_RELU>, dim3(tiles), dim3(512), GX_LDS_BYTES, st, a, wx);
   } else {
diff --git a/self-diagnosing-gan_amd/csrc/gemm_x3_halo.h b/self-diagnosing-gan_amd/csrc/gemm_x3_halo.h
--- /dev/null
+++ b/self-diagnosing-gan_amd/csrc/gemm_x3_halo.h
@@ -0,0 +1,43 @@
+#pragma once
+
+#if defined(__HIPCC__)
+#define GXR_HD __host__ __device__ inline
+#else
+#define GXR_HD inline
+#endif
+
+namespace diagan {
+
+constexpr int GXR_HW = 8;
+constexpr int GXR_HALO = GXR_HW + 2;
+constexpr int GXR_BORDER = 4 * GXR_HW + 4;
+constexpr int GXR_WSTAGE = 3 * 64 * 40;
+constexpr int GXR_LDS_MAX = 160 * 1024;
+
+GXR_HD int gxr_pix_pitch(int Ci) { return Ci + 8; }
+GXR_HD int gxr_row_pitch(int Ci) {
+  const int slots = GXR_HALO * (Ci / 8 + 1);
+  return (slots + ((8 - slots) & 15)) * 8;
+}
+GXR_HD int gxr_plane(int Ci) { return GXR_HALO * gxr_row_pitch(Ci); }
+GXR_HD long gxr_lds_bytes(int Ci) { return (4L * GXR_WSTAGE + 3L * gxr_plane(Ci)) * 2; }
+
+GXR_HD int gxr_halo_pixel(int pix, int r, int s, int dr, int off) {
+  return ((pix >> 3) + 1 + off + r * dr) * GXR_HALO + (pix & 7) + 1 + off + s * dr;
+}
+GXR_HD int gxr_halo_off(int pix, int r, int s, int dr, int off, int Ci) {
+  return ((pix >> 3) + 1 + off + r * dr) * gxr_row_pitch(Ci) + ((pix & 7) + 1 + off + s * dr) * gxr_pix_pitch(Ci);
+}
+GXR_HD void gxr_border_pixel(int i, int& hy, int& hx) {
+  if (i < GXR_HALO) { hy = 0; hx = i; }
+  else if (i < 2 * GXR_HALO) { hy = GXR_HALO - 1; hx = i - GXR_HALO; }
+  else if (i < 2 * GXR_HALO + GXR_HW) { hy = i - 2 * GXR_HALO + 1; hx = 0; }
+  else { hy = i - 2 * GXR_HALO - GXR_HW + 1; hx = GXR_HALO - 1; }
+}
+
+GXR_HD bool gxr_shape_ok(int B, int Hi, int Wi, int Ci, int Ho, int Wo, int R, int S, int dr, int off) {
+  return R == 3 && S == 3 && ((dr == 1 && off == -1) || (dr == -1 && off == 1)) && Hi == GXR_HW && Wi == GXR_HW && Ho == GXR_HW &&
+         Wo == GXR_HW && Ci > 0 && (Ci & 31) == 0 && gxr_lds_bytes(Ci) <= GXR_LDS_MAX && (long)B * 64 * Ci * 4 < (1L << 31);
+}
+
+}
diff --git a/self-diagnosing-gan_amd/diagan/_native/conv_x3_abi.py b/self-diagnosing-gan_amd/diagan/_native/conv_x3_abi.py
--- /dev/null
+++ b/self-diagnosing-gan_amd/diagan/_native/conv_x3_abi.py
@@ -0,0 +1,35 @@
+import os
+
+from diagan import _native as nat
+from diagan._native import parse_header
+
+HEADER_PATH = os.path.join(os.path.dirname(nat.HEADER_PATH), "diagan_conv_x3.h")
+
+_sigs = None
+_bound = {}
+
+
+def signatures():
+    global _sigs
+    if _sigs is None:
+        if not os.path.exists(HEADER_PATH):
+            raise RuntimeError(f"diagan_conv_x3.h not found at {HEADER_PATH}: the ctypes signatures are read from it "
+                               "(the package runs from a checkout of the repository).")
+        with open(HEADER_PATH) as f:
+            _sigs = parse_header(f.read())
+    return _sigs
+
+
+def fn(name):
+    f = _bound.get(name)
+    if f is None:
+        f = getattr(nat.lib(), name)
+        f.restype, f.argtypes = signatures()[name]
+        _bound[name] = f
+    return f
+
+
+def call(name, *args):
+    rc = fn(name)(*args)
+    if rc != 0:
+        raise RuntimeError(f"{name} failed ({rc}): {nat.last_error()}")
diff --git a/self-diagnosing-gan_amd/diagan/ops/conv.py b/self-diagnosing-gan_amd/diagan/ops/conv.py
--- a/self-diagnosing-gan_amd/diagan/ops/conv.py
+++ b/self-diagnosing-gan_amd/diagan/ops/conv.py
@@ -199,6 +199,28 @@
     nat.call("diagan_conv_gemm_set_x3b", -1 if on is None else (1 if on else 0))
 
 
+def set_gemm_x3_resident(on):
+    from diagan._native import conv_x3_abi as xnat
+    xnat.call("diagan_conv_gemm_set_x3_resident", -1 if on is None else (1 if on else 0))
+
+
+def last_x3_form():
+    from diagan._native import conv_x3_abi as xnat
+    return xnat.fn("diagan_conv_gemm_last_x3_form")()
+
+
+def gemm_x3_resident_ok(geom, B, Hi, Wi, dgrad=False, mode=PRO_NONE):
+    from diagan._native import conv_x3_abi as xnat
+    if dgrad:
+        sy, dr, off, up = geom.dgrad_params()
+        return bool(xnat.fn("diagan_conv_gemm_x3_resident_ok")(B, Hi, Wi, geom.Co, Hi, Wi, geom.Ci, geom.R, geom.S, sy, dr, off, up,
+                                                               geom.Kd, mode))
+    sy, dr, off, up = geom.fwd_params()
+    Ho, Wo = geom.out_hw(Hi, Wi)
+    return bool(xnat.fn("diagan_conv_gemm_x3_resident_ok")(B, Hi, Wi, geom.Ci, Ho, Wo, geom.Co, geom.R, geom.S, sy, dr, off, up,
+                                                           geom.Kp, mode))
+
+
 def set_gemm_x3b(on):
     nat.call("diagan_conv_gemm_set_x3b", -1 if on is None else (1 if on else 0))
 
@@ -233,11 +255,11 @@
 
 class ConvOpts(_ct.Structure):
     _fields_ = [(n, _ct.c_int32) for n in ("wino", "wino4", "wino4x", "gemm_x3", "gemm_x3b", "splitk_fused", "force_ksplit", "tune")] + \
-               [("tickets", _ct.c_void_p), ("ticket_slots", _ct.c_int64)]
+               [("tickets", _ct.c_void_p), ("ticket_slots", _ct.c_int64), ("gemm_x3_resident", _ct.c_int32)]
 
 
 def next_opts(tickets=None, **fields):
-    o = ConvOpts(-1, -1, -1, -1, -1, -1, 0, -1, None, 0)
+    o = ConvOpts(-1, -1, -1, -1, -1, -1, 0, -1, None, 0, -1)
     for k, v in fields.items():
         setattr(o, k, int(v))
     if tickets is not None:
@@ -252,7 +274,7 @@
 
 
 def _opts_key(o):
-    return tuple(getattr(o, n) for n, _ in ConvOpts._fields_[:8])
+    return tuple(getattr(o, n) for n, _ in ConvOpts._fields_[:8]) + (o.gemm_x3_resident,)
 
 
 def _without_wino(o):
```

Measured after the change: 5287, median of 6. 1.0% higher.
